# alexcoca/DistributedKernelShap

Measured on AMD Instinct MI355X. Metric: explanations/sec (2560 inst, 100-sample background), higher is better.
Workload: dtype fp32; 1 GPU; model=adult-logreg (12 groups, D=50, n_out=2, logit link), global_batch=2560, background=100, nsamples=default(2M+2048), parallelism=dp1, device=cuda

## Files before the change

distributedkernelshap_amd/config.py:

```python
from __future__ import annotations

import dataclasses
from dataclasses import dataclass, field
from typing import Any, Dict, List, Optional, Union

__all__ = [
    "EngineConfig",
    "DistributedConfig",
    "ServeConfig",
    "BenchConfig",
    "KernelConfig",
    "Config",
]


@dataclass
class EngineConfig:

    link: str = "logit"
    seed: int = 0
    nsamples: Optional[int] = None
    l1_reg: Union[str, int, float, None] = "auto"
    device: str = "auto"
    chunk_rows: int = 1 << 20


@dataclass
class DistributedConfig:

    n_workers: Optional[int] = None
    batch_size: int = 1
    actor_cpu_fraction: float = 1.0
    backend: str = "auto"
    mp_context: Optional[str] = None

    def to_opts(self) -> Dict[str, Any]:
        d = {
            "n_workers": self.n_workers,
            "batch_size": self.batch_size,
            "actor_cpu_fraction": self.actor_cpu_fraction,
        }
        if self.mp_context:
            d["mp_context"] = self.mp_context
        return d


@dataclass
class ServeConfig:
    host: str = "127.0.0.1"
    port: int = 8800
    replicas: int = 1
    max_batch_size: int = 64
    max_wait_ms: float = 2.0


@dataclass
class KernelConfig:

    wls_mode: str = "auto"
    fused_predict: bool = True
    predict_dtype: str = "fp32"
    packed_mma: str = "auto"
    synth_chunk_rows: int = 1 << 21
    l1_device: bool = True
    module_autocast: str = "off"
    module_channels_last: bool = True


@dataclass
class BenchConfig:
    instances: int = 2560
    background: int = 100
    nruns: int = 5
    steps: int = 5
    warmup: int = 2
    batch_sizes: List[int] = field(default_factory=lambda: [1, 5, 10])
    results_dir: str = "results"
    assets_dir: str = "assets"


@dataclass
class Config:
    engine: EngineConfig = field(default_factory=EngineConfig)
    distributed: DistributedConfig = field(default_factory=DistributedConfig)
    serve: ServeConfig = field(default_factory=ServeConfig)
    kernels: KernelConfig = field(default_factory=KernelConfig)
    bench: BenchConfig = field(default_factory=BenchConfig)

    @classmethod
    def from_dict(cls, d: Dict[str, Any]) -> "Config":
        cfg = cls()
        for section, values in d.items():
            if not hasattr(cfg, section):
                raise KeyError(f"unknown config section '{section}'")
            sub = getattr(cfg, section)
            names = {f.name for f in dataclasses.fields(sub)}
            for k, v in values.items():
                if k not in names:
                    raise KeyError(f"unknown key '{section}.{k}'")
                setattr(sub, k, v)
        return cfg

    @classmethod
    def from_toml(cls, path: str) -> "Config":
        import tomli

        with open(path, "rb") as f:
            return cls.from_dict(tomli.load(f))

    def to_dict(self) -> Dict[str, Any]:
        return dataclasses.asdict(self)
```

distributedkernelshap_amd/ops/gpu_engine.py:

```python
from __future__ import annotations

import logging
from typing import List, Optional

import numpy as np

from . import load_extension
from ..core.sampler import CoalitionPlan

logger = logging.getLogger(__name__)

import os as _os
import time as _time

_TIMING = _os.environ.get("KSHAP_TIMING", "") == "1"


class _StageTimer:

    def __init__(self, torch_mod, enabled, sink=None):
        self.t = torch_mod
        self.enabled = enabled or sink is not None
        self.sink = sink
        self.last = _time.perf_counter() if self.enabled else 0.0
# ... 590 lines not shown
                else t.tensor(varying, dtype=t.int64, device=self.device))
        xv = self._x_part(X_dev)[:, vidx]
        bgv = self.bg_part[:, vidx]
        return xv.permute(0, 2, 1)[:, :, :, None] - bgv.permute(2, 1, 0)[None]

    def _ey_fused_linear(self, masks, X_dev, varying, vidx_t=None):
        t = self.torch
        b, s, m = masks.shape
        mpad = max(4, (m + 3) // 4 * 4)
        npad = (self.N + 15) // 16 * 16
        if vidx_t is None:
            vidx_t = t.tensor(varying, dtype=t.int64, device=self.device)
        act, oimg = self._act_oimg()
        diff = self._buf(f"diff{m}", (b, oimg, mpad, npad), zeroed=True)
        self.ext.build_diff_f32(
            self._x_part_img(X_dev, act), self._bg_part_img(act), vidx_t, diff
        )
        base = t.zeros(oimg, npad, device=self.device)
        base[:, : self.N] = self._base_img(act)
        wbg = t.zeros(npad, device=self.device)
        wbg[: self.N] = self.bg_w
        ey = self._buf("ey", (b, s, self.n_out))
        self.ext.fused_predict_linear(masks, diff, base, wbg, ey, act)
        return ey

    def _act_oimg(self):
        act = self.linear["act"]
        if act == 2 and self.n_out == 2:
            return 3, 1
        return act, self.n_out

    def _x_part_img(self, X_dev, act):
        xp = self._x_part(X_dev)
        if act == 3:
            return (xp[:, :, 1:2] - xp[:, :, 0:1]).contiguous()
        return xp

    def _bg_part_img(self, act):
        if act == 3:
            if not hasattr(self, "_bg_part_d"):
                self._bg_part_d = (
                    self.bg_part[:, :, 1:2] - self.bg_part[:, :, 0:1]
                ).contiguous()
            return self._bg_part_d
        return self.bg_part

    def _base_img(self, act):
        if act == 3:
            return (self.baseN[:, 1] - self.baseN[:, 0])[None, :]
        return self.baseN.T

    def _ey_fused_bf16(self, masks, X_dev, varying, vidx_t=None, packed=None):
        t = self.torch
        b, s, m = masks.shape
        npad = (self.N + 15) // 16 * 16
        split = 2 if self.engine.kernels.predict_dtype == "bf16x2" else 1
        if packed is not None:
            self.ext.pack_masks(masks, packed)
        if vidx_t is None:
            vidx_t = t.tensor(varying, dtype=t.int64, device=self.device)
        act, oimg = self._act_oimg()
        diffB = self._buf(
            f"diffB{m}", (b, split, oimg, npad, 40), t.bfloat16, zeroed=True
        )
        self.ext.build_diff_bf16(
            self._x_part_img(X_dev, act), self._bg_part_img(act), vidx_t, diffB
        )
        base = t.zeros(oimg, npad, device=self.device)
        base[:, : self.N] = self._base_img(act)
        wbg = t.zeros(npad, device=self.device)
        wbg[: self.N] = self.bg_w
        ey = self._buf("ey", (b, s, self.n_out))
        self.ext.fused_predict_bf16(masks, diffB, base, wbg, ey, act)
        return ey

    def _ey_fused_tiled(self, masks, X_dev, varying, vidx_t=None):
        t = self.torch
        b, s, m = masks.shape
        mpad = max(16, (m + 15) // 16 * 16)
        npad = (self.N + 15) // 16 * 16
        if vidx_t is None:
            vidx_t = t.tensor(varying, dtype=t.int64, device=self.device)
        act, oimg = self._act_oimg()
        diff = self._buf(f"difft{m}", (b, oimg, mpad, npad), zeroed=True)
        self.ext.build_diff_f32(
            self._x_part_img(X_dev, act), self._bg_part_img(act), vidx_t, diff
        )
        base = t.zeros(oimg, npad, device=self.device)
        base[:, : self.N] = self._base_img(act)
        wbg = t.zeros(npad, device=self.device)
        wbg[: self.N] = self.bg_w
        n_ntiles = (npad + 127) // 128
        partial = self._buf("ftpart", (b, n_ntiles, s, self.n_out))
        ey = self._buf("ey", (b, s, self.n_out))
        self.ext.fused_predict_tiled(masks, diff, base, wbg, partial, ey, act)
        return ey

    def _ey_linear_f64(self, masks, X_dev, varying, s_chunk=2048):
        t = self.torch
        b, s, m = masks.shape
        W = self.linear["W"].double()
        bias = self.linear["b"].double()
        bg = self.bg.double()
        X64 = X_dev.double()
        contrib_x = X64[:, :, None] * W.T[None, :, :]
        x_part = t.zeros(b, self.n_groups, self.n_out, dtype=t.float64,
                         device=self.device)
        x_part.index_add_(1, self.col_group, contrib_x)
        contrib_b = bg[:, :, None] * W.T[None, :, :]
        bg_part = t.zeros(self.N, self.n_groups, self.n_out, dtype=t.float64,
                          device=self.device)
        bg_part.index_add_(1, self.col_group, contrib_b)
        vidx = t.tensor(varying, dtype=t.int64, device=self.device)
        diff = (x_part[:, vidx].permute(0, 2, 1)[:, :, :, None]
                - bg_part[:, vidx].permute(2, 1, 0)[None])
        diff = diff.permute(0, 2, 3, 1).reshape(b, m, self.N * self.n_out)
        base = bg @ W.T + bias
        wbg64 = self.bg_w.double()
        ey = t.empty(b, s, self.n_out, dtype=t.float64, device=self.device)
        for lo in range(0, s, s_chunk):
            hi = min(lo + s_chunk, s)
            logits = t.bmm(masks[:, lo:hi].double(), diff)
            logits = logits.view(b, hi - lo, self.N, self.n_out) + base[None, None]
            a = self.linear["act"]
            if a == 1:
                p = t.sigmoid(logits)
            elif a == 2:
                p = t.softmax(logits, dim=-1)
            else:
                p = logits
            ey[:, lo:hi] = t.einsum("bsno,n->bso", p, wbg64)
        return ey

    def _ey_fused_tiled_bf16(self, masks, X_dev, varying, vidx_t=None):
        t = self.torch
        b, s, m = masks.shape
        mpad = max(32, (m + 31) // 32 * 32)
        npad = (self.N + 15) // 16 * 16
        if vidx_t is None:
            vidx_t = t.tensor(varying, dtype=t.int64, device=self.device)
        act, oimg = self._act_oimg()
        split = 2 if self.engine.kernels.predict_dtype == "bf16x2" else 1
        diffb = self._buf(
            f"difftb{m}", (b, split, oimg, npad, mpad), t.bfloat16,
            zeroed=True,
        )
        self.ext.build_diff_bf16_tiled(
            self._x_part_img(X_dev, act), self._bg_part_img(act), vidx_t,
            diffb,
        )
        base = t.zeros(oimg, npad, device=self.device)
        base[:, : self.N] = self._base_img(act)
        wbg = t.zeros(npad, device=self.device)
        wbg[: self.N] = self.bg_w
        n_ntiles = (npad + 127) // 128
        partial = self._buf("ftpart", (b, n_ntiles, s, self.n_out))
        ey = self._buf("ey", (b, s, self.n_out))
        self.ext.fused_predict_tiled_bf16(
            masks, diffb, base, wbg, partial, ey, act
        )
        return ey

    def _ey_linear_torch(self, masks, X_dev, varying, s_chunk=4096):
        t = self.torch
        b, s, m = masks.shape
        diff = self._diff_tensor(X_dev, varying)
        diff = diff.permute(0, 2, 3, 1).reshape(b, m, self.N * self.n_out)
        ey = t.empty(b, s, self.n_out, device=self.device)
        for lo in range(0, s, s_chunk):
            hi = min(lo + s_chunk, s)
            logits = t.bmm(masks[:, lo:hi].float(), diff)
            logits = logits.view(b, hi - lo, self.N, self.n_out) + self.baseN[None, None]
            a = self.linear["act"]
            if a == 1:
                p = t.sigmoid(logits)
            elif a == 2:
                p = t.softmax(logits, dim=-1)
            else:
                p = logits
            ey[:, lo:hi] = t.einsum("bsno,n->bso", p, self.bg_w)
        return ey

    def _ey_torch_module(self, masks, X_dev, varying, chunk_rows=None):
        t = self.torch
        b, s, m = masks.shape
        if chunk_rows is None:
            chunk_rows = max(self.N, self.engine.kernels.synth_chunk_rows or 1 << 19)
        chunk_rows = min(chunk_rows, max(self.N, (1 << 29) // max(1, self.D)))
        chunk_rows = min(chunk_rows, b * s * self.N)
        ey = t.empty(b, s, self.n_out, device=self.device)
        vmap = np.full(self.n_groups, m, dtype=np.int64)
        for i, g in enumerate(varying):
            vmap[g] = i
        mfull = self._buf("mfull", (b, s, m + 1), t.uint8)
        mfull.zero_()
        mfull[:, :, :m] = masks
        colg = t.tensor(
            vmap[self.engine._col_group].astype(np.int32), device=self.device
        )
        sdt = (t.bfloat16 if self.engine.kernels.module_autocast == "bf16"
               else t.float32)
        rows_per_inst = s * self.N
        if rows_per_inst <= chunk_rows:
            g_inst = max(1, min(b, chunk_rows // rows_per_inst))
            buf = self._buf("synth", (g_inst * rows_per_inst, self.D), sdt)
            for lo in range(0, b, g_inst):
                hi = min(lo + g_inst, b)
                rows = (hi - lo) * rows_per_inst
                out = buf[:rows]
                self.ext.synth_chunk(mfull, X_dev, self.bg, colg, out, lo, hi, 0, s)
                y = self._predict_rows(out)
                ey[lo:hi] = t.einsum(
                    "csno,n->cso",
                    y.view(hi - lo, s, self.N, self.n_out),
                    self.bg_w,
                )
        else:
            s_chunk = max(1, chunk_rows // self.N)
            buf = self._buf("synth", (s_chunk * self.N, self.D), sdt)
            for bi in range(b):
                for lo in range(0, s, s_chunk):
                    hi = min(lo + s_chunk, s)
                    rows = (hi - lo) * self.N
                    out = buf[:rows]
                    self.ext.synth_chunk(
                        mfull, X_dev, self.bg, colg, out, bi, bi + 1, lo, hi
                    )
                    y = self._predict_rows(out)
                    y = y.view(hi - lo, self.N, self.n_out)
                    ey[bi, lo:hi] = t.einsum("cno,n->co", y, self.bg_w)
        return ey


    def _packed_ok(self, m, plan, l1_reg) -> bool:
        kc = self.engine.kernels
        return (
            self.linear is not None
            and kc.predict_dtype == "fp32"
            and kc.fused_predict
            and kc.wls_mode in ("auto", "mfma")
            and 2 <= m <= 64
            and (self.N + 15) // 16 * 16 <= 128
            and self.n_out in (1, 2, 4)
            and (m - 1) + self.n_out <= 16
            and not self._l1_active(plan, l1_reg)
        )

    def _packed_consts(self):
        c = getattr(self, "_packed_c", None)
        if c is None:
            t = self.torch
            act, oimg = self._act_oimg()
            npad = (self.N + 15) // 16 * 16
            base = t.zeros(oimg, npad, device=self.device)
            base[:, : self.N] = self._base_img(act)
            wbg = t.zeros(npad, device=self.device)
            wbg[: self.N] = self.bg_w
            lfnull64 = self._link(self.fnull.double()).contiguous()
            c = {
                "act": act, "oimg": oimg, "npad": npad, "base": base,
                "wbg": wbg, "lfnull64": lfnull64,
                "lfnull": lfnull64.float().contiguous(),
                "bgp": self._bg_part_img(act).contiguous(),
                "link": 0 if self.link_name == "identity" else 1,
            }
            self._packed_c = c
        return c

    def _packed_plan(self, plan):
        t = self.torch
        key = ("packed", plan.m, plan.nsamples)
        ent = self._enum_cache.get(key)
        if ent is None:
            ne = plan.enum_masks.shape[0]
            enum_packed = t.empty(1, ne, dtype=t.int64, device=self.device)
            if ne > 0:
                enum = t.tensor(plan.enum_masks, dtype=t.uint8,
                                device=self.device)
                self.ext.pack_masks(enum[None].contiguous(), enum_packed)
            kw = t.empty(plan.nsamples, dtype=t.float32, device=self.device)
            kw[:ne] = t.tensor(plan.enum_weights, dtype=t.float32,
                               device=self.device)
            if plan.n_random > 0:
                kw[ne:] = plan.weight_left / plan.n_random
            cdf = t.tensor(
                np.cumsum(plan.random_size_probs).astype(np.float32),
                device=self.device,
            )
            szs = t.tensor(plan.random_sizes.astype(np.int32),
                           device=self.device)
            ent = (enum_packed[0].contiguous(), kw, cdf, szs)
            self._enum_cache[key] = ent
        return ent

    def _packed_mma(self):
        mode = self.engine.kernels.packed_mma
        try:
            return {"auto": -1, "f32": 0, "split": 1}[mode]
        except KeyError:
            raise ValueError(
                f"packed_mma must be 'auto', 'f32' or 'split', got {mode!r}"
            ) from None

    def _packed_pipeline(self, X_dev, plan, vidx_t, ids_dev, phi_full,
                         timer=None):
        t = self.torch
        b = X_dev.shape[0]
        m, s = plan.m, plan.nsamples
        c = self._packed_consts()
        enum_packed, kw, cdf, szs = self._packed_plan(plan)
        mpad = max(4, (m + 3) // 4 * 4)
        packed = self._buf("packed", (b, s), t.int64)
        self.ext.fill_masks_packed(
            packed, enum_packed, plan.n_random, cdf, szs,
            int(np.floor((m - 1) / 2.0)), int(self.engine.seed), ids_dev, m,
        )
        if timer is not None:
            timer.mark("masks")
        diff = self._buf(f"diffp{m}", (b, c["oimg"], mpad, c["npad"]))
        total = self._buf("totalp", (b, self.n_out))
        self.ext.linear_prepare(
            X_dev, self.linear["W"], self.linear["b"], self.col_group, vidx_t,
            c["bgp"], c["lfnull64"], diff, total, c["act"], c["link"],
        )
        ey = self._buf("ey", (b, s, self.n_out))
        self.ext.fused_predict_linear_packed(
            packed, diff, c["base"], c["wbg"], ey, c["act"], c["link"],
            c["lfnull"], self._packed_mma(),
        )
        if timer is not None:
            timer.mark("predict")
        self.ext.wls_solve_packed(packed, kw, ey, total, vidx_t, phi_full)
        if timer is not None:
            timer.mark("wls")


    def _fused_body(self, X_dev, plan, varying, vidx_t, ids_dev, phi_full):
        t = self.torch
        b = X_dev.shape[0]
        m = len(varying)
        if self._packed_ok(m, plan, False):
            self._packed_pipeline(X_dev, plan, vidx_t, ids_dev, phi_full)
            return
        fx = self._predict_rows_f64(X_dev)
        lfx = self._link(fx)
        lfnull64 = self._link(self.fnull.double())
        total = (lfx - lfnull64[None, :]).float().contiguous()
        lfnull = lfnull64.float()
        masks, kw = self._device_masks(plan, np.arange(b), ids_dev=ids_dev)
        kc = self.engine.kernels
        packed = self._buf("packed", (b, plan.nsamples), t.int64)
        self.ext.pack_masks(masks, packed)
        if (kc.predict_dtype in ("bf16", "bf16x2") and m <= 32
                and self.n_out in (1, 2, 4)):
            ey = self._ey_fused_bf16(masks, X_dev, varying, vidx_t, packed=None)
        else:
            ey = self._ey_fused_linear(masks, X_dev, varying, vidx_t)
        if self.link_name == "identity":
            ey_adj = ey.sub_(lfnull[None, None, :])
        else:
            ey.clamp_(_EPS, 1.0 - _EPS)
            ey.log_().sub_(t.log1p(-t.exp(ey)))
            ey_adj = ey.sub_(lfnull[None, None, :])
        phi = self._buf("phi", (b, m, self.n_out))
        self.ext.wls_solve(masks, kw, ey_adj, total, phi, packed)
        phi_full.zero_()
        phi_full[:, vidx_t] = phi

    def _graph_explain(self, X_dev, plan, varying, instance_offset,
                       as_tensor=False):
        t = self.torch
        b = X_dev.shape[0]
        key = (b, plan.nsamples, varying.tobytes())
        entry = self._graphs.get(key)
        if entry is None:
            hits = self._graph_hits.get(key, 0) + 1
            self._graph_hits[key] = hits
            if hits < self._graph_min_hits or len(self._graphs) >= 8:
                return None
            try:
                vidx_t = t.tensor(varying, dtype=t.int64, device=self.device)
                x_static = self._buf("Xg", (b, self.D))
                ids_static = self._buf("idsg", (b,), t.int32)
                phi_full = t.zeros(
                    b, self.n_groups, self.n_out, device=self.device
                )
                x_static.copy_(X_dev)
                ids_static.copy_(
                    t.arange(instance_offset, instance_offset + b,
                             dtype=t.int32, device=self.device)
                )
                side = t.cuda.Stream()
                side.wait_stream(t.cuda.current_stream())
                with t.cuda.stream(side):
                    self._fused_body(
                        x_static, plan, varying, vidx_t, ids_static, phi_full
                    )
                t.cuda.current_stream().wait_stream(side)
                graph = t.cuda.CUDAGraph()
                with t.cuda.graph(graph):
                    self._fused_body(
                        x_static, plan, varying, vidx_t, ids_static, phi_full
                    )
                entry = (graph, x_static, ids_static, phi_full, vidx_t)
                self._graphs[key] = entry
            except Exception as e:
                logger.warning(
                    "hipGraph capture failed (%r); continuing eagerly", e
                )
                self._graphs_enabled = False
                return None
        graph, x_static, ids_static, phi_full, _ = entry
        if x_static.data_ptr() != X_dev.data_ptr():
            x_static.copy_(X_dev)
        ids_static.copy_(
            t.arange(instance_offset, instance_offset + b, dtype=t.int32,
                     device=self.device)
        )
        graph.replay()
        if as_tensor:
            return phi_full.clone()
        out = phi_full.double().cpu().numpy()
        return [np.ascontiguousarray(out[:, :, o]) for o in range(self.n_out)]

    _CHUNK_BYTES = 2 << 30

    def _instances_per_chunk(self, nsamples: Optional[int],
                             l1_reg="auto") -> int:
        from ..core.sampler import default_nsamples

        s = nsamples or default_nsamples(max(2, self.n_groups))
        g = self.n_groups
        if g >= 2 and self._packed_ok(g, self.engine._plan(g, nsamples),
                                      l1_reg):
            npad = (self.N + 15) // 16 * 16
            per_inst = (s * (8 + 4 * self.n_out)
                        + 4 * self.n_out * (g + 3) * npad + (1 << 14))
            return max(1, self._CHUNK_BYTES // per_inst)
        npad = (self.N + 15) // 16 * 16
        n_ntiles = (npad + 127) // 128
        per_inst = s * (g + 8 + 4 + 4 * self.n_out) + (1 << 14)
        if g > 64 or npad > 128:
            per_inst += s * 4 * self.n_out * n_ntiles
            mpad = max(4, (g + 3) // 4 * 4)
            per_inst += 4 * mpad * npad * max(1, self.n_out)
            per_inst += 8 * g * (g + self.n_out) * 2
        if self.mlp_fused:
            h1 = self.mlp["pack"]["hpad"][0]
            per_inst += 8 * g * (self.D + 2 * h1) + 4 * h1 * (g + 31)
        if self.trees_kernel == "bits":
            per_inst += self.trees["pack"]["n_trees"] * (8 + 64 * 9)
        return max(1, self._CHUNK_BYTES // per_inst)

    def shap_values(
        self,
        X: np.ndarray,
        nsamples: Optional[int] = None,
        l1_reg="auto",
        instance_offset: int = 0,
        as_tensor: bool = False,
    ) -> List[np.ndarray]:
        t = self.torch
        b_total = X.shape[0]
        chunk = self._instances_per_chunk(nsamples, l1_reg)
        if b_total > chunk:
            if as_tensor:
                out = t.empty(
                    b_total, self.n_groups, self.n_out, device=self.device,
                    dtype=(t.float64
                           if self.engine.kernels.predict_dtype == "fp64"
                           else t.float32),
                )
                for lo in range(0, b_total, chunk):
                    hi = min(lo + chunk, b_total)
                    out[lo:hi] = self.shap_values(
                        X[lo:hi], nsamples=nsamples, l1_reg=l1_reg,
                        instance_offset=instance_offset + lo, as_tensor=True,
                    )
                return out
            parts = [
                self.shap_values(
                    X[lo : lo + chunk], nsamples=nsamples, l1_reg=l1_reg,
                    instance_offset=instance_offset + lo,
                )
                for lo in range(0, b_total, chunk)
            ]
            return [
                np.concatenate([p[o] for p in parts], axis=0)
                for o in range(self.n_out)
            ]
        timer = _StageTimer(t, _TIMING, sink=self.trace)
        if t.is_tensor(X):
            b = X.shape[0]
            if X.is_cuda:
                X_dev = X.float()
            else:
                X_dev = self._spec_x_static(b, X.shape[1])
                if X_dev is None:
                    X_dev = self._buf("X", (b, X.shape[1]))
                X_dev.copy_(X, non_blocking=True)
        else:
            X = np.ascontiguousarray(X, dtype=np.float64)
            b = X.shape[0]
            X_dev = t.tensor(X, dtype=t.float32, device=self.device)
        timer.mark("h2d")

        fp64 = self.engine.kernels.predict_dtype == "fp64"
        if (
            self._graphs_enabled
            and not fp64
            and self._spec is not None
            and self.linear is not None
            and self.n_groups <= 62
        ):
            sk0, skey, sm = self._spec
            sb, sns, soff = skey[0], skey[1], skey[3]
            entry = self._graphs.get((skey[0], skey[1], skey[2]))
            spec_plan = self.engine._plan(sm, nsamples) if entry is not None else None
            if (entry is not None and sb == b and spec_plan.nsamples == sns
                    and not self._l1_active(spec_plan, l1_reg)
                    and soff == int(instance_offset)):
                graph, x_static, ids_static, gphi, _ = entry
                if x_static.data_ptr() != X_dev.data_ptr():
                    x_static.copy_(X_dev)
                graph.replay()
                _, probe = self._varying_probe(x_static)
                staged = None if as_tensor else self._phi_stage_enqueue(gphi)
                pc = probe.cpu()
                timer.mark("spec")
                if bool(pc[0]) and int(pc[1]) == sk0:
                    if as_tensor:
                        return gphi.clone()
                    timer.mark("d2h")
                    return [
                        np.ascontiguousarray(staged[:, :, o], dtype=np.float64)
                        for o in range(self.n_out)
                    ]
                self._spec = None

        X64_dev = None
        f64c = next((c for c in (self.mlp, self.trees, self.km)
                     if c is not None), None)
        if fp64 and f64c is not None:
            X64_dev = (X.to(self.device).double() if t.is_tensor(X)
                       else t.tensor(X, dtype=t.float64, device=self.device))
        fx = self._predict_rows_f64(
            X_dev if X64_dev is None else X64_dev)
        lfx = self._link(fx)
        lfnull64 = self._link(
            self.fnull.double() if X64_dev is None else f64c["fnull64"])
        total_all = (lfx - lfnull64[None, :])
        if not fp64:
            total_all = total_all.float()
        lfnull = lfnull64.float()

        phi_full = t.zeros(b, self.n_groups, self.n_out, device=self.device,
                           dtype=t.float64 if fp64 else t.float32)

        if self.n_groups <= 62:
            keys, probe = self._varying_probe(X_dev)
            probe = probe.cpu()
            timer.mark("varying")
            if bool(probe[0]):
                key0 = int(probe[1])
                uniq = np.array(
                    [[(key0 >> g) & 1 for g in range(self.n_groups)]],
                    dtype=bool,
                )
                inverse = np.zeros(b, dtype=np.int64)
            else:
                ks = keys.cpu().numpy()
                kuniq, inverse = np.unique(ks, return_inverse=True)
                uniq = ((kuniq[:, None] >> np.arange(self.n_groups)) & 1
                        ).astype(bool)
        else:
            vmat = self._varying_matrix_dev(X_dev).cpu().numpy()
            timer.mark("varying")
            uniq, inverse = np.unique(vmat, axis=0, return_inverse=True)
        timer.mark("bucket")

        kc = self.engine.kernels
        if self._graphs_enabled and not fp64 and uniq.shape[0] == 1 \
                and self.linear is not None \
                and kc.fused_predict and kc.wls_mode in ("auto", "mfma"):
            varying0 = np.nonzero(uniq[0])[0]
            m0 = len(varying0)
            if m0 >= 2:
                plan0 = self.engine._plan(m0, nsamples)
                mpad0 = max(4, (m0 + 3) // 4 * 4)
                npad0 = (self.N + 15) // 16 * 16
                if (
                    mpad0 <= 64
                    and npad0 <= 128
                    and self.n_out in (1, 2, 4)
                    and not self._l1_active(plan0, l1_reg)
                ):
                    out = self._graph_explain(
                        X_dev, plan0, varying0, instance_offset,
                        as_tensor=as_tensor,
                    )
                    if out is not None:
                        key0 = 0
                        for g in varying0:
                            key0 |= 1 << int(g)
                        self._spec = (
                            key0,
                            (b, plan0.nsamples, varying0.tobytes(),
                             int(instance_offset)),
                            m0,
                        )
                        timer.mark("graph")
                        return out

        for u in range(uniq.shape[0]):
            varying = np.nonzero(uniq[u])[0]
            m = len(varying)
            ids = np.nonzero(inverse == u)[0]
            ids_t = t.tensor(ids, dtype=t.int64, device=self.device)
            if m == 0:
                continue
            if m == 1:
                phi_full[ids_t, int(varying[0])] = total_all[ids_t]
                continue
            plan = self.engine._plan(m, nsamples)
            gids = ids + instance_offset
            if not fp64 and self._packed_ok(m, plan, l1_reg):
                nb = len(ids)
# ... 364 lines not shown
```

distributedkernelshap_amd/ops/hip/bindings.cpp:

```cpp
#include <torch/extension.h>
#include <ATen/hip/HIPContext.h>
#include <c10/hip/HIPStream.h>

#include <cstdint>

extern "C" void launch_fill_random_masks(
    uint8_t* masks, int B, int S, int M, int ne, int n_random,
    const float* cdf, const int* sizes, int n_sizes, int num_paired,
    uint32_t seed, const int32_t* inst_ids, hipStream_t stream);

extern "C" int launch_fused_predict_linear(
    const uint8_t* masksU, const float* diff, const float* base, const float* wbg,
    float* ey, int B, int S, int M, int Mpad, int Npad, int n_out, int act,
    hipStream_t stream);

extern "C" void launch_synth_chunk(
    const uint8_t* masks, const float* x, const float* bg, const int* col_group,
    void* out, int out_bf16, int S, int M, int N, int D, int b_lo, int b_hi,
    int s_lo, int s_hi, hipStream_t stream);

extern "C" void launch_pack_masks(
    const uint8_t* masks, uint64_t* packed, int B, int S, int M,
    hipStream_t stream);

extern "C" int launch_fused_predict_bf16(
    const uint8_t* masksU, const uint16_t* diffB,
    const float* base, const float* wbg, float* ey, int B, int S, int M,
    int Npad, int n_out, int act, int split, hipStream_t stream);

extern "C" void launch_build_diff_f32(
    const float* xp, const float* bgp, const int64_t* vidx, float* out,
    int B, int G, int O, int N, int m, int Mpad, int Npad, hipStream_t stream);

extern "C" void launch_build_diff_bf16(
    const float* xp, const float* bgp, const int64_t* vidx, uint16_t* out,
    int B, int G, int O, int N, int m, int Npad, int split, hipStream_t stream);

extern "C" int launch_wls_solve(
    const uint8_t* masks, const uint64_t* packed, const float* kw,
    const float* ey_adj, const float* total, float* phi, int B, int S, int M,
    int n_out, hipStream_t stream);

extern "C" void launch_pack_masks_words(
    const uint8_t* masks, uint64_t* packed, int B, int S, int M, int W,
    hipStream_t stream);

extern "C" int launch_wls_gram(
    const uint64_t* packed, const float* kw, const float* ey_adj,
    const float* total, double* A64, double* rhs64, int B, int S, int M,
    int W, int n_out, hipStream_t stream);

extern "C" int launch_fused_predict_tiled(
    const uint8_t* masksU, const float* diff, const float* base,
    const float* wbg, float* partial, float* ey, int B, int S, int M,
    int Mpad, int Npad, int n_out, int act, hipStream_t stream);

extern "C" void launch_build_diff_bf16_tiled(
    const float* xp, const float* bgp, const int64_t* vidx, uint16_t* out,
    int B, int G, int O, int N, int m, int Mpad, int Npad, int split,
    hipStream_t stream);

extern "C" int launch_fused_predict_tiled_bf16(
    const uint8_t* masksU, const uint16_t* diffB, const float* base,
    const float* wbg, float* partial, float* ey, int B, int S, int M,
    int Mpad, int Npad, int n_out, int act, int split, hipStream_t stream);

extern "C" int launch_fill_masks_packed(
    uint64_t* packed, const uint64_t* enum_packed, int B, int S, int M, int ne,
    int n_random, const float* cdf, const int* sizes, int n_sizes,
    int num_paired, uint32_t seed, const int32_t* inst_ids, hipStream_t stream);

extern "C" int launch_linear_prepare(
    const float* X, const float* W, const float* bias,
    const int64_t* col_group, const int64_t* vidx, const float* bgp,
    const double* lfnull64, float* diff, float* total, int B, int D, int G,
    int N, int m, int Mpad, int Npad, int n_out, int act, int link,
    hipStream_t stream);

extern "C" int launch_fused_predict_linear_packed(
    const uint64_t* packed, const float* diff, const float* base,
    const float* wbg, const float* lfnull, float* ey, int B, int S, int Mpad,
    int Npad, int n_out, int act, int link, hipStream_t stream, int mma);

extern "C" int launch_wls_solve_packed(
    const uint64_t* packed, const float* kw, const float* ey_adj,
    const float* total, const int64_t* vidx, float* phi_full, int B, int S,
    int M, int n_out, int G, hipStream_t stream);

extern "C" int launch_varying_probe(
    const float* X, const float* bg_min, const float* bg_max,
    const float* tol_min, const float* tol_max, const int64_t* col_group,
    int64_t* keys, int64_t* probe, int B, int D, int G, hipStream_t stream);

extern "C" int launch_fused_predict_mlp(
    const uint8_t* masks, const void* xp1, const void* bgp1n,
    const float* base1, const void* const* hw, const float* const* hb,
    const int* H, int nhid, const void* wout, const float* bout,
    const float* wbg, float* ey, int B, int S, int M, int Mpad, int N,
    int n_out, int act, int hidden_act, int is_bf16, int nsplit,
    hipStream_t stream);

extern "C" int launch_fused_predict_trees(
    const uint8_t* masks, const int* vmap, const int64_t* dx, const int64_t* dbg,
    const uint8_t* child, const int* meta, const float* leaves,
    const int* grp_off, const int* grp_id, const int64_t* grp_mask,
    const float* base, const float* wbg, float* ey, float scale,
    int B, int S, int Mv, int N, int T, int G, int E, int L, int C,
    int max_internal, int n_out, int act, int leaf_mode, hipStream_t stream);

extern "C" int launch_fused_predict_trees_walk(
    const uint8_t* masks, const int* vmap, const float* x, const float* bg,
    const int* nodes, const int* roots, const float* leaves, const float* base,
    const float* wbg, float* ey, float scale,
    int B, int S, int Mv, int N, int D, int G, int T, int R, int L,
    int max_depth, int n_out, int act, int leaf_mode,
    const unsigned* cat_left, int C, hipStream_t stream);

extern "C" int launch_fused_predict_kernelmachine(
    const uint8_t* masks, const float* xp, const float* bgpn,
    const float* base, const float* alpha, const float* icpt,
    const float* wbg, float* ey, int B, int S, int M, int Mpad, int N,
    int Vpad, int n_out, int act, int kernel, float gamma, float coef0,
    int degree, hipStream_t stream);

namespace {

#define CHECK_DEV(t) TORCH_CHECK((t).is_cuda() && (t).is_contiguous(), #t " must be a contiguous device tensor")

hipStream_t current_stream() {
    return c10::hip::getCurrentHIPStream().stream();
}

void fill_random_masks(
    torch::Tensor masks, int64_t ne, int64_t n_random,
    torch::Tensor cdf, torch::Tensor sizes, int64_t num_paired, int64_t seed,
    torch::Tensor inst_ids) {
    CHECK_DEV(masks); CHECK_DEV(cdf); CHECK_DEV(sizes); CHECK_DEV(inst_ids);
    TORCH_CHECK(masks.dtype() == torch::kUInt8, "masks must be uint8");
    TORCH_CHECK(masks.dim() == 3, "masks must be (B,S,M)");
    TORCH_CHECK(inst_ids.dtype() == torch::kInt32, "inst_ids must be int32");
    int B = masks.size(0), S = masks.size(1), M = masks.size(2);
    TORCH_CHECK(inst_ids.size(0) == B, "inst_ids length");
    TORCH_CHECK(M <= 256, "fill_random_masks supports M <= 256");
    launch_fill_random_masks(
        masks.data_ptr<uint8_t>(), B, S, M, (int)ne, (int)n_random,
        cdf.data_ptr<float>(), sizes.data_ptr<int>(), (int)cdf.size(0),
        (int)num_paired, (uint32_t)seed, inst_ids.data_ptr<int32_t>(),
        current_stream());
}

void fused_predict_linear(
    torch::Tensor masks, torch::Tensor diff, torch::Tensor base,
    torch::Tensor wbg, torch::Tensor ey, int64_t act) {
    CHECK_DEV(masks); CHECK_DEV(diff); CHECK_DEV(base); CHECK_DEV(wbg); CHECK_DEV(ey);
    TORCH_CHECK(masks.dtype() == torch::kUInt8, "masks must be u8 (B,S,M)");
    int B = masks.size(0), S = masks.size(1), M = masks.size(2);
    int Mpad = diff.size(2), Npad = diff.size(3);
    int n_out = ey.size(2);
    int oimg = (act == 3) ? 1 : n_out;
    TORCH_CHECK(diff.size(1) == oimg, "diff image count vs act");
    TORCH_CHECK(M <= Mpad, "M vs Mpad");
    TORCH_CHECK(ey.size(0) == B && ey.size(1) == S, "ey shape");
    TORCH_CHECK(base.size(0) == oimg && base.size(1) == Npad, "base shape");
    TORCH_CHECK(wbg.size(0) == Npad, "wbg shape");
    int rc = launch_fused_predict_linear(
        masks.data_ptr<uint8_t>(), diff.data_ptr<float>(), base.data_ptr<float>(),
        wbg.data_ptr<float>(), ey.data_ptr<float>(), B, S, M, Mpad, Npad,
        n_out, (int)act, current_stream());
    TORCH_CHECK(rc == 0, "fused_predict_linear: unsupported shape (Mpad<=64, Npad%16==0, Npad<=128, n_out in {1,2,4})");
}

void synth_chunk(
    torch::Tensor masks, torch::Tensor x, torch::Tensor bg,
    torch::Tensor col_group, torch::Tensor out, int64_t b_lo, int64_t b_hi,
    int64_t s_lo, int64_t s_hi) {
    CHECK_DEV(masks); CHECK_DEV(x); CHECK_DEV(bg); CHECK_DEV(col_group); CHECK_DEV(out);
    int S = masks.size(1), M = masks.size(2);
    int N = bg.size(0), D = bg.size(1);
    TORCH_CHECK(out.size(0) == (b_hi - b_lo) * (s_hi - s_lo) * N && out.size(1) == D,
                "out shape");
    const bool bf16 = out.dtype() == torch::kBFloat16;
    TORCH_CHECK(bf16 || out.dtype() == torch::kFloat32,
                "out must be float32 or bfloat16");
    launch_synth_chunk(
        masks.data_ptr<uint8_t>(), x.data_ptr<float>(), bg.data_ptr<float>(),
        col_group.data_ptr<int>(),
        bf16 ? (void*)out.data_ptr<at::BFloat16>()
             : (void*)out.data_ptr<float>(),
        bf16 ? 1 : 0, S, M, N, D,
        (int)b_lo, (int)b_hi, (int)s_lo, (int)s_hi, current_stream());
}

void wls_solve(
    torch::Tensor masks, torch::Tensor kw, torch::Tensor ey_adj,
    torch::Tensor total, torch::Tensor phi,
    c10::optional<torch::Tensor> packed) {
    CHECK_DEV(masks); CHECK_DEV(kw); CHECK_DEV(ey_adj); CHECK_DEV(total); CHECK_DEV(phi);
    int B = masks.size(0), S = masks.size(1), M = masks.size(2);
    int n_out = ey_adj.size(2);
    TORCH_CHECK(phi.size(0) == B && phi.size(1) == M && phi.size(2) == n_out, "phi shape");
    const uint64_t* pk = nullptr;
    if (packed.has_value()) {
        CHECK_DEV(packed.value());
        TORCH_CHECK(packed->size(0) == B && packed->size(1) == S, "packed shape");
        pk = reinterpret_cast<const uint64_t*>(packed->data_ptr<int64_t>());
    }
    int rc = launch_wls_solve(
        masks.data_ptr<uint8_t>(), pk, kw.data_ptr<float>(), ey_adj.data_ptr<float>(),
        total.data_ptr<float>(), phi.data_ptr<float>(), B, S, M, n_out,
        current_stream());
    TORCH_CHECK(rc == 0, "wls_solve: unsupported shape (2<=M<=64, n_out<=8)");
}

void pack_masks(torch::Tensor masks, torch::Tensor packed) {
    CHECK_DEV(masks); CHECK_DEV(packed);
    TORCH_CHECK(masks.dtype() == torch::kUInt8, "masks must be u8");
    int B = masks.size(0), S = masks.size(1), M = masks.size(2);
    TORCH_CHECK(M <= 64, "pack_masks supports M <= 64");
    TORCH_CHECK(packed.size(0) == B && packed.size(1) == S, "packed shape");
    launch_pack_masks(
        masks.data_ptr<uint8_t>(),
        reinterpret_cast<uint64_t*>(packed.data_ptr<int64_t>()),
        B, S, M, current_stream());
}

#define CHECK_F32(t) TORCH_CHECK((t).dtype() == torch::kFloat32, #t " must be float32")
#define CHECK_I64(t) TORCH_CHECK((t).dtype() == torch::kInt64, #t " must be int64")

void fill_masks_packed(
    torch::Tensor packed, torch::Tensor enum_packed, int64_t n_random,
    torch::Tensor cdf, torch::Tensor sizes, int64_t num_paired, int64_t seed,
    torch::Tensor inst_ids, int64_t M) {
    CHECK_DEV(packed); CHECK_DEV(enum_packed); CHECK_DEV(cdf); CHECK_DEV(sizes);
    CHECK_DEV(inst_ids);
    CHECK_I64(packed); CHECK_I64(enum_packed); CHECK_F32(cdf);
    TORCH_CHECK(sizes.dtype() == torch::kInt32, "sizes must be int32");
    TORCH_CHECK(inst_ids.dtype() == torch::kInt32, "inst_ids must be int32");
    TORCH_CHECK(packed.dim() == 2 && enum_packed.dim() == 1,
                "packed must be (B,S), enum_packed (ne,)");
    int B = packed.size(0), S = packed.size(1), ne = enum_packed.size(0);
    TORCH_CHECK(inst_ids.dim() == 1 && inst_ids.size(0) == B, "inst_ids length");
    TORCH_CHECK(n_random >= 0 && ne + n_random == S, "ne + n_random must equal S");
    TORCH_CHECK(cdf.dim() == 1 && sizes.dim() == 1
                && cdf.size(0) == sizes.size(0), "cdf vs sizes");
    TORCH_CHECK(n_random == 0 || cdf.size(0) >= 1, "empty size table");
    int rc = launch_fill_masks_packed(
        reinterpret_cast<uint64_t*>(packed.data_ptr<int64_t>()),
        reinterpret_cast<const uint64_t*>(enum_packed.data_ptr<int64_t>()),
        B, S, (int)M, ne, (int)n_random, cdf.data_ptr<float>(),
        sizes.data_ptr<int>(), (int)cdf.size(0), (int)num_paired,
        (uint32_t)seed, inst_ids.data_ptr<int32_t>(), current_stream());
    TORCH_CHECK(rc == 0, "fill_masks_packed: unsupported shape (1<=M<=64)");
}

void linear_prepare(
    torch::Tensor X, torch::Tensor W, torch::Tensor bias,
    torch::Tensor col_group, torch::Tensor vidx, torch::Tensor bgp,
    torch::Tensor lfnull64, torch::Tensor diff, torch::Tensor total,
    int64_t act, int64_t link) {
    CHECK_DEV(X); CHECK_DEV(W); CHECK_DEV(bias); CHECK_DEV(col_group);
    CHECK_DEV(vidx); CHECK_DEV(bgp); CHECK_DEV(lfnull64); CHECK_DEV(diff);
    CHECK_DEV(total);
    CHECK_F32(X); CHECK_F32(W); CHECK_F32(bias); CHECK_F32(bgp); CHECK_F32(diff);
    CHECK_F32(total); CHECK_I64(col_group); CHECK_I64(vidx);
    TORCH_CHECK(lfnull64.dtype() == torch::kFloat64, "lfnull64 must be float64");
    TORCH_CHECK(X.dim() == 2 && W.dim() == 2 && bgp.dim() == 3 && diff.dim() == 4
                && total.dim() == 2 && vidx.dim() == 1, "operand ranks");
    int B = X.size(0), D = X.size(1), n_out = W.size(0);
    int N = bgp.size(0), G = bgp.size(1), OI = bgp.size(2), m = vidx.size(0);
    int Mpad = diff.size(2), Npad = diff.size(3);
    TORCH_CHECK(W.size(1) == D && bias.numel() == n_out
                && col_group.numel() == D && lfnull64.numel() == n_out,
                "W (n_out,D), b (n_out), col_group (D), lfnull64 (n_out)");
    TORCH_CHECK(OI == (act == 3 ? 1 : n_out), "background image count vs act");
    TORCH_CHECK(diff.size(0) == B && diff.size(1) == OI, "diff (B,OI,Mpad,Npad)");
    TORCH_CHECK(total.size(0) == B && total.size(1) == n_out, "total (B,n_out)");
    TORCH_CHECK(link == 0 || link == 1, "link must be 0 or 1");
    int rc = launch_linear_prepare(
        X.data_ptr<float>(), W.data_ptr<float>(), bias.data_ptr<float>(),
        col_group.data_ptr<int64_t>(), vidx.data_ptr<int64_t>(),
        bgp.data_ptr<float>(), lfnull64.data_ptr<double>(),
        diff.data_ptr<float>(), total.data_ptr<float>(), B, D, G, N, m, Mpad,
        Npad, n_out, (int)act, (int)link, current_stream());
    TORCH_CHECK(rc == 0, "linear_prepare: unsupported shape (m<=Mpad, m<=64, "
                         "N<=Npad, n_out<=8, act 3 needs n_out==2)");
}

void fused_predict_linear_packed(
    torch::Tensor packed, torch::Tensor diff, torch::Tensor base,
    torch::Tensor wbg, torch::Tensor ey, int64_t act, int64_t link,
    c10::optional<torch::Tensor> lfnull, int64_t mma) {
    CHECK_DEV(packed); CHECK_DEV(diff); CHECK_DEV(base); CHECK_DEV(wbg); CHECK_DEV(ey);
    CHECK_I64(packed); CHECK_F32(diff); CHECK_F32(base); CHECK_F32(wbg); CHECK_F32(ey);
    TORCH_CHECK(packed.dim() == 2 && diff.dim() == 4 && ey.dim() == 3
                && base.dim() == 2, "operand ranks");
    int B = packed.size(0), S = packed.size(1);
    int Mpad = diff.size(2), Npad = diff.size(3);
    int n_out = ey.size(2);
    int oimg = (act == 3) ? 1 : n_out;
    TORCH_CHECK(diff.size(0) == B && diff.size(1) == oimg, "diff (B,oimg,Mpad,Npad) vs act");
    TORCH_CHECK(ey.size(0) == B && ey.size(1) == S, "ey shape");
    TORCH_CHECK(base.size(0) == oimg && base.size(1) == Npad, "base shape");
    TORCH_CHECK(wbg.numel() == Npad, "wbg shape");
    const float* lf = nullptr;
    if (lfnull.has_value()) {
        CHECK_DEV(lfnull.value()); CHECK_F32(lfnull.value());
        TORCH_CHECK(lfnull->numel() == n_out, "lfnull must be (n_out,)");
        lf = lfnull->data_ptr<float>();
    }
    TORCH_CHECK(link == 0 || (link == 1 && lf != nullptr),
                "link must be 0, or 1 with lfnull given");
    TORCH_CHECK(mma >= -1 && mma <= 1,
                "mma must be -1 (auto), 0 (fp32 MFMA) or 1 (split bf16 MFMA)");
    int rc = launch_fused_predict_linear_packed(
        reinterpret_cast<const uint64_t*>(packed.data_ptr<int64_t>()),
        diff.data_ptr<float>(), base.data_ptr<float>(), wbg.data_ptr<float>(),
        lf, ey.data_ptr<float>(), B, S, Mpad, Npad, n_out, (int)act, (int)link,
        current_stream(), (int)mma);
    TORCH_CHECK(rc == 0, "fused_predict_linear_packed: unsupported shape "
                         "(Mpad%4==0, Mpad<=64, Npad%16==0, Npad<=128, n_out in "
                         "{1,2,4}, operand images within 64 KiB of LDS)");
}

void wls_solve_packed(
    torch::Tensor packed, torch::Tensor kw, torch::Tensor ey_adj,
    torch::Tensor total, torch::Tensor vidx, torch::Tensor phi_full) {
    CHECK_DEV(packed); CHECK_DEV(kw); CHECK_DEV(ey_adj); CHECK_DEV(total);
    CHECK_DEV(vidx); CHECK_DEV(phi_full);
    CHECK_I64(packed); CHECK_F32(kw); CHECK_F32(ey_adj); CHECK_F32(total);
    CHECK_I64(vidx); CHECK_F32(phi_full);
    TORCH_CHECK(packed.dim() == 2 && ey_adj.dim() == 3 && phi_full.dim() == 3
                && vidx.dim() == 1 && total.dim() == 2, "operand ranks");
    int B = packed.size(0), S = packed.size(1), M = vidx.size(0);
    int n_out = ey_adj.size(2), G = phi_full.size(1);
    TORCH_CHECK(kw.numel() == S, "kw must be (S,)");
    TORCH_CHECK(ey_adj.size(0) == B && ey_adj.size(1) == S, "ey_adj shape");
    TORCH_CHECK(total.size(0) == B && total.size(1) == n_out, "total shape");
    TORCH_CHECK(phi_full.size(0) == B && phi_full.size(2) == n_out, "phi_full shape");
    int rc = launch_wls_solve_packed(
        reinterpret_cast<const uint64_t*>(packed.data_ptr<int64_t>()),
        kw.data_ptr<float>(), ey_adj.data_ptr<float>(), total.data_ptr<float>(),
        vidx.data_ptr<int64_t>(), phi_full.data_ptr<float>(), B, S, M, n_out,
        G, current_stream());
    TORCH_CHECK(rc == 0, "wls_solve_packed: unsupported shape (2<=M<=G, "
                         "(M-1)+n_out<=16)");
}

void varying_probe(
    torch::Tensor X, torch::Tensor bg_min, torch::Tensor bg_max,
    torch::Tensor tol_min, torch::Tensor tol_max, torch::Tensor col_group,
    int64_t n_groups, torch::Tensor keys, torch::Tensor probe) {
    CHECK_DEV(X); CHECK_DEV(bg_min); CHECK_DEV(bg_max); CHECK_DEV(tol_min);
    CHECK_DEV(tol_max); CHECK_DEV(col_group); CHECK_DEV(keys); CHECK_DEV(probe);
    CHECK_F32(X); CHECK_F32(bg_min); CHECK_F32(bg_max); CHECK_F32(tol_min);
    CHECK_F32(tol_max); CHECK_I64(col_group); CHECK_I64(keys); CHECK_I64(probe);
    TORCH_CHECK(X.dim() == 2, "X must be (B,D)");
    const int64_t B = X.size(0), D = X.size(1);
    TORCH_CHECK(B >= 1 && D >= 1 && B <= 0x7fffffffLL && D <= 0x7fffffffLL,
                "X must be (B,D) with B, D >= 1");
    TORCH_CHECK(bg_min.numel() == D && bg_max.numel() == D
                && tol_min.numel() == D && tol_max.numel() == D
                && col_group.numel() == D,
                "bg_min, bg_max, tol_min, tol_max, col_group must be (D,)");
    TORCH_CHECK(keys.numel() == B, "keys must be (B,)");
    TORCH_CHECK(probe.numel() == 2, "probe must be (2,)");
    int rc = launch_varying_probe(
        X.data_ptr<float>(), bg_min.data_ptr<float>(), bg_max.data_ptr<float>(),
        tol_min.data_ptr<float>(), tol_max.data_ptr<float>(),
        col_group.data_ptr<int64_t>(), keys.data_ptr<int64_t>(),
        probe.data_ptr<int64_t>(), (int)B, (int)D, (int)n_groups,
        current_stream());
    TORCH_CHECK(rc == 0, "varying_probe: unsupported shape (1 <= n_groups <= 62)");
}

void fused_predict_bf16(
    torch::Tensor masks, torch::Tensor diffB, torch::Tensor base,
    torch::Tensor wbg, torch::Tensor ey, int64_t act) {
    CHECK_DEV(masks); CHECK_DEV(diffB); CHECK_DEV(base); CHECK_DEV(wbg); CHECK_DEV(ey);
    TORCH_CHECK(masks.dtype() == torch::kUInt8 && diffB.dtype() == torch::kBFloat16);
    int B = masks.size(0), S = masks.size(1), M = masks.size(2);
    int split = diffB.size(1), Npad = diffB.size(3);
    int n_out = ey.size(2);
    TORCH_CHECK(diffB.size(2) == ((act == 3) ? 1 : n_out), "diffB image count vs act");
    TORCH_CHECK(diffB.size(0) == B && diffB.size(4) == 40, "diffB (B,split,o,Npad,40)");
    TORCH_CHECK(ey.size(0) == B && ey.size(1) == S, "ey shape");
    int rc = launch_fused_predict_bf16(
        masks.data_ptr<uint8_t>(),
        reinterpret_cast<const uint16_t*>(diffB.data_ptr<at::BFloat16>()),
        base.data_ptr<float>(), wbg.data_ptr<float>(), ey.data_ptr<float>(),
        B, S, M, Npad, n_out, (int)act, split, current_stream());
    TORCH_CHECK(rc == 0, "fused_predict_bf16: unsupported shape (M<=32, Npad<=128, n_out in {1,2,4}, split in {1,2})");
}

void build_diff_f32(torch::Tensor xp, torch::Tensor bgp, torch::Tensor vidx,
                    torch::Tensor out) {
    CHECK_DEV(xp); CHECK_DEV(bgp); CHECK_DEV(vidx); CHECK_DEV(out);
    int B = xp.size(0), G = xp.size(1), O = xp.size(2);
    int N = bgp.size(0), m = vidx.size(0);
    int Mpad = out.size(2), Npad = out.size(3);
    TORCH_CHECK(out.size(0) == B && out.size(1) == O && m <= Mpad && N <= Npad);
    launch_build_diff_f32(
        xp.data_ptr<float>(), bgp.data_ptr<float>(), vidx.data_ptr<int64_t>(),
        out.data_ptr<float>(), B, G, O, N, m, Mpad, Npad, current_stream());
}

void build_diff_bf16(torch::Tensor xp, torch::Tensor bgp, torch::Tensor vidx,
                     torch::Tensor out) {
    CHECK_DEV(xp); CHECK_DEV(bgp); CHECK_DEV(vidx); CHECK_DEV(out);
    TORCH_CHECK(out.dtype() == torch::kBFloat16 && out.size(4) == 40);
    int B = xp.size(0), G = xp.size(1), O = xp.size(2);
    int N = bgp.size(0), m = vidx.size(0);
    int split = out.size(1), Npad = out.size(3);
    TORCH_CHECK(out.size(0) == B && out.size(2) == O && N <= Npad && m <= 32);
    launch_build_diff_bf16(
        xp.data_ptr<float>(), bgp.data_ptr<float>(), vidx.data_ptr<int64_t>(),
        reinterpret_cast<uint16_t*>(out.data_ptr<at::BFloat16>()), B, G, O, N,
        m, Npad, split, current_stream());
}

void pack_masks_words(torch::Tensor masks, torch::Tensor packed) {
    CHECK_DEV(masks); CHECK_DEV(packed);
    TORCH_CHECK(masks.dtype() == torch::kUInt8, "masks must be u8");
    TORCH_CHECK(packed.dim() == 3, "packed must be (B,S,W)");
    int B = masks.size(0), S = masks.size(1), M = masks.size(2);
    int W = packed.size(2);
    TORCH_CHECK(packed.size(0) == B && packed.size(1) == S, "packed shape");
    TORCH_CHECK(W * 64 >= M, "packed word count vs M");
    launch_pack_masks_words(
        masks.data_ptr<uint8_t>(),
        reinterpret_cast<uint64_t*>(packed.data_ptr<int64_t>()),
        B, S, M, W, current_stream());
}

void wls_gram(
    torch::Tensor packed, torch::Tensor kw, torch::Tensor ey_adj,
    torch::Tensor total, torch::Tensor A64, torch::Tensor rhs64) {
    CHECK_DEV(packed); CHECK_DEV(kw); CHECK_DEV(ey_adj); CHECK_DEV(total);
    CHECK_DEV(A64); CHECK_DEV(rhs64);
    TORCH_CHECK(packed.dim() == 3, "packed must be (B,S,W)");
    TORCH_CHECK(A64.dtype() == torch::kFloat64 && rhs64.dtype() == torch::kFloat64);
    int B = packed.size(0), S = packed.size(1), W = packed.size(2);
    int mm = A64.size(1), n_out = ey_adj.size(2);
    TORCH_CHECK(A64.size(0) == B && A64.size(2) == mm, "A64 shape");
    TORCH_CHECK(rhs64.size(0) == B && rhs64.size(1) == mm
                && rhs64.size(2) == n_out, "rhs64 shape");
    TORCH_CHECK(W * 64 >= mm + 1, "packed word count vs M");
    int rc = launch_wls_gram(
        reinterpret_cast<const uint64_t*>(packed.data_ptr<int64_t>()),
        kw.data_ptr<float>(), ey_adj.data_ptr<float>(),
        total.data_ptr<float>(), A64.data_ptr<double>(),
        rhs64.data_ptr<double>(), B, S, mm + 1, W, n_out, current_stream());
    TORCH_CHECK(rc == 0, "wls_gram: unsupported shape (M<=513, n_out<=8)");
}

void fused_predict_tiled(
    torch::Tensor masks, torch::Tensor diff, torch::Tensor base,
    torch::Tensor wbg, torch::Tensor partial, torch::Tensor ey, int64_t act) {
    CHECK_DEV(masks); CHECK_DEV(diff); CHECK_DEV(base); CHECK_DEV(wbg);
    CHECK_DEV(partial); CHECK_DEV(ey);
    TORCH_CHECK(masks.dtype() == torch::kUInt8, "masks must be u8 (B,S,M)");
    int B = masks.size(0), S = masks.size(1), M = masks.size(2);
    int Mpad = diff.size(2), Npad = diff.size(3);
    int n_out = ey.size(2);
    int oimg = (act == 3) ? 1 : n_out;
    int nacc = n_out;
    int n_ntiles = (Npad + 127) / 128;
    TORCH_CHECK(diff.size(1) == oimg, "diff image count vs act");
    TORCH_CHECK(M <= Mpad, "M vs Mpad");
    TORCH_CHECK(ey.size(0) == B && ey.size(1) == S, "ey shape");
    TORCH_CHECK(base.size(0) == oimg && base.size(1) == Npad, "base shape");
    TORCH_CHECK(wbg.size(0) == Npad, "wbg shape");
    TORCH_CHECK(partial.size(0) == B && partial.size(1) == n_ntiles
                && partial.size(2) == S && partial.size(3) == nacc,
                "partial shape (B, n_ntiles, S, nacc)");
    int rc = launch_fused_predict_tiled(
        masks.data_ptr<uint8_t>(), diff.data_ptr<float>(),
        base.data_ptr<float>(), wbg.data_ptr<float>(),
        partial.data_ptr<float>(), ey.data_ptr<float>(), B, S, M, Mpad,
        Npad, n_out, (int)act, current_stream());
    TORCH_CHECK(rc == 0, "fused_predict_tiled: unsupported shape "
                         "(Mpad%4==0, Npad%16==0, n_out in {1,2,4})");
}

void build_diff_bf16_tiled(torch::Tensor xp, torch::Tensor bgp,
                           torch::Tensor vidx, torch::Tensor out) {
    CHECK_DEV(xp); CHECK_DEV(bgp); CHECK_DEV(vidx); CHECK_DEV(out);
    TORCH_CHECK(out.dtype() == torch::kBFloat16 && out.dim() == 5,
                "out must be bf16 (B,split,O,Npad,Mpad)");
    int B = xp.size(0), G = xp.size(1), O = xp.size(2);
    int N = bgp.size(0), mcount = vidx.size(0);
    int split = out.size(1), Npad = out.size(3), Mpad = out.size(4);
    TORCH_CHECK(out.size(0) == B && out.size(2) == O && N <= Npad
                && mcount <= Mpad);
    launch_build_diff_bf16_tiled(
        xp.data_ptr<float>(), bgp.data_ptr<float>(), vidx.data_ptr<int64_t>(),
        reinterpret_cast<uint16_t*>(out.data_ptr<at::BFloat16>()), B, G, O, N,
        mcount, Mpad, Npad, split, current_stream());
}

void fused_predict_tiled_bf16(
    torch::Tensor masks, torch::Tensor diffB, torch::Tensor base,
    torch::Tensor wbg, torch::Tensor partial, torch::Tensor ey, int64_t act) {
    CHECK_DEV(masks); CHECK_DEV(diffB); CHECK_DEV(base); CHECK_DEV(wbg);
    CHECK_DEV(partial); CHECK_DEV(ey);
    TORCH_CHECK(masks.dtype() == torch::kUInt8
                && diffB.dtype() == torch::kBFloat16);
    int B = masks.size(0), S = masks.size(1), M = masks.size(2);
    int split = diffB.size(1), Npad = diffB.size(3), Mpad = diffB.size(4);
    int n_out = ey.size(2);
    int oimg = (act == 3) ? 1 : n_out;
    int n_ntiles = (Npad + 127) / 128;
    TORCH_CHECK(diffB.size(2) == oimg, "diffB image count vs act");
    TORCH_CHECK(ey.size(0) == B && ey.size(1) == S, "ey shape");
    TORCH_CHECK(base.size(0) == oimg && base.size(1) == Npad, "base shape");
    TORCH_CHECK(wbg.size(0) == Npad, "wbg shape");
    TORCH_CHECK(partial.size(0) == B && partial.size(1) == n_ntiles
                && partial.size(2) == S && partial.size(3) == n_out,
                "partial shape");
    TORCH_CHECK((size_t)split * oimg * 128 * 40 * 2 <= 64 * 1024,
                "bf16 tiled LDS footprint (split*oimg too large)");
    int rc = launch_fused_predict_tiled_bf16(
        masks.data_ptr<uint8_t>(),
        reinterpret_cast<const uint16_t*>(diffB.data_ptr<at::BFloat16>()),
        base.data_ptr<float>(), wbg.data_ptr<float>(),
        partial.data_ptr<float>(), ey.data_ptr<float>(), B, S, M, Mpad, Npad,
        n_out, (int)act, split, current_stream());
    TORCH_CHECK(rc == 0, "fused_predict_tiled_bf16: unsupported shape "
                         "(Mpad%32==0, Npad%16==0, n_out in {1,2,4})");
}

void fused_predict_mlp(
    torch::Tensor masks, torch::Tensor xp1, torch::Tensor bgp1n,
    torch::Tensor base1, std::vector<torch::Tensor> hidden_w,
    std::vector<torch::Tensor> hidden_b, torch::Tensor wout,
    torch::Tensor bout, torch::Tensor wbg, torch::Tensor ey, int64_t act,
    int64_t hidden_act) {
    static const char* envelope =
        "fused_predict_mlp: outside the supported envelope (1-3 relu hidden "
        "layers of padded width <= 256, n_out <= 8, M <= Mpad <= 64, widths "
        "padded to 16 (fp32) / 32 (bf16))";
    CHECK_DEV(masks); CHECK_DEV(xp1); CHECK_DEV(bgp1n); CHECK_DEV(base1);
    CHECK_DEV(wout); CHECK_DEV(bout); CHECK_DEV(wbg); CHECK_DEV(ey);
    TORCH_CHECK(masks.dtype() == torch::kUInt8 && masks.dim() == 3,
                "masks must be u8 (B,S,M)");
    const bool bf16 = xp1.dtype() == torch::kBFloat16;
    TORCH_CHECK(bf16 || xp1.dtype() == torch::kFloat32,
                "operand images must be float32 or bfloat16");
    const auto wdt = xp1.dtype();
    TORCH_CHECK(hidden_w.size() == hidden_b.size(), "hidden_w vs hidden_b");
    TORCH_CHECK(hidden_w.size() + 1 <= 3, envelope);
    const int nhid = (int)hidden_w.size() + 1;
    TORCH_CHECK(xp1.dim() == 3 && bgp1n.dim() == 3 && base1.dim() == 2
                && wout.dim() == 3 && ey.dim() == 3, "operand ranks");
    int B = masks.size(0), S = masks.size(1), M = masks.size(2);
    int H[3] = {(int)xp1.size(1), 0, 0};
    int Mpad = xp1.size(2), N = bgp1n.size(0), n_out = ey.size(2);
    TORCH_CHECK(xp1.size(0) == B, "xp1 must be (B,H1,Mpad)");
    TORCH_CHECK(bgp1n.dtype() == wdt && bgp1n.size(1) == H[0]
                && bgp1n.size(2) == Mpad, "bgp1n must be (N,H1,Mpad)");
    TORCH_CHECK(base1.dtype() == torch::kFloat32 && base1.size(0) == N
                && base1.size(1) == H[0], "base1 must be f32 (N,H1)");
    const void* hw[2] = {nullptr, nullptr};
    const float* hb[2] = {nullptr, nullptr};
    for (int l = 1; l < nhid; ++l) {
        const torch::Tensor& w = hidden_w[l - 1];
        const torch::Tensor& bb = hidden_b[l - 1];
        CHECK_DEV(w); CHECK_DEV(bb);
        TORCH_CHECK(w.dtype() == wdt && w.dim() == 2 && w.size(1) == H[l - 1],
                    "hidden weight must be (H_out, H_in) in the operand dtype");
        H[l] = w.size(0);
        TORCH_CHECK(bb.dtype() == torch::kFloat32 && bb.dim() == 1
                    && bb.size(0) == H[l], "hidden bias must be f32 (H_out)");
        hw[l - 1] = w.data_ptr();
        hb[l - 1] = bb.data_ptr<float>();
    }
    const int nsplit = wout.size(0);
    TORCH_CHECK(wout.dtype() == wdt && wout.size(1) == 16
                && wout.size(2) == H[nhid - 1], "wout must be (nsplit,16,H_last)");
    TORCH_CHECK(bout.dtype() == torch::kFloat32 && bout.numel() == 16,
                "bout must be f32 (16)");
    TORCH_CHECK(wbg.dtype() == torch::kFloat32 && wbg.numel() == N, "wbg must be f32 (N)");
    TORCH_CHECK(ey.dtype() == torch::kFloat32 && ey.size(0) == B
                && ey.size(1) == S, "ey must be f32 (B,S,n_out)");
    int rc = launch_fused_predict_mlp(
        masks.data_ptr<uint8_t>(), xp1.data_ptr(), bgp1n.data_ptr(),
        base1.data_ptr<float>(), hw, hb, H, nhid, wout.data_ptr(),
        bout.data_ptr<float>(), wbg.data_ptr<float>(), ey.data_ptr<float>(),
        B, S, M, Mpad, N, n_out, (int)act, (int)hidden_act, bf16 ? 1 : 0,
        nsplit, current_stream());
    TORCH_CHECK(rc != -2, "fused_predict_mlp: LDS size attribute rejected");
    TORCH_CHECK(rc == 0, envelope);
}

void fused_predict_trees(
    torch::Tensor masks, torch::Tensor vmap, torch::Tensor dx,
    torch::Tensor dbg, torch::Tensor child, torch::Tensor meta,
    torch::Tensor leaves, torch::Tensor grp_off, torch::Tensor grp_id,
    torch::Tensor grp_mask, torch::Tensor base, double scale,
    torch::Tensor wbg, torch::Tensor ey, int64_t act, int64_t leaf_mode,
    int64_t max_internal) {
    static const char* envelope =
        "fused_predict_trees: outside the supported envelope (1-1024 trees of "
        "at most 64 internal nodes each, n_out <= 8, 128 B per tree plus 2 B "
        "per internal node within 160 KiB of LDS)";
    CHECK_DEV(masks); CHECK_DEV(vmap); CHECK_DEV(dx); CHECK_DEV(dbg);
    CHECK_DEV(child); CHECK_DEV(meta); CHECK_DEV(leaves); CHECK_DEV(grp_off);
    CHECK_DEV(grp_id); CHECK_DEV(grp_mask); CHECK_DEV(base); CHECK_DEV(wbg);
    CHECK_DEV(ey);
    TORCH_CHECK(masks.dtype() == torch::kUInt8 && masks.dim() == 3,
                "masks must be u8 (B,S,Mv)");
    TORCH_CHECK(ey.dtype() == torch::kFloat32 && ey.dim() == 3,
                "ey must be f32 (B,S,n_out)");
    const int B = masks.size(0), S = masks.size(1), Mv = masks.size(2);
    const int n_out = ey.size(2);
    TORCH_CHECK(ey.size(0) == B && ey.size(1) == S, "ey must be f32 (B,S,n_out)");
    TORCH_CHECK(vmap.dtype() == torch::kInt32 && vmap.dim() == 1,
                "the group table must be int32 (G)");
    TORCH_CHECK(dx.dtype() == torch::kInt64 && dx.dim() == 2 && dx.size(0) == B,
                "dx must be int64 (B,T)");
    const int T = dx.size(1);
    TORCH_CHECK(dbg.dtype() == torch::kInt64 && dbg.dim() == 2
                && dbg.size(1) == T, "dbg must be int64 (N,T)");
    const int N = dbg.size(0);
    TORCH_CHECK(child.dtype() == torch::kUInt8 && child.dim() == 2
                && child.size(1) == 2, "child must be u8 (C,2)");
    TORCH_CHECK(meta.dtype() == torch::kInt32 && meta.dim() == 2
                && meta.size(0) == T && meta.size(1) == 4,
                "meta must be int32 (T,4)");
    TORCH_CHECK(leaf_mode == 0 || leaf_mode == 1, "leaf_mode must be 0 or 1");
    TORCH_CHECK(leaves.dtype() == torch::kFloat32
                && (leaf_mode == 0 ? leaves.dim() == 1
                                   : (leaves.dim() == 2 && leaves.size(1) == n_out)),
                "leaves must be f32 (L) for scalar or (L,n_out) for vector leaves");
    TORCH_CHECK(grp_off.dtype() == torch::kInt32 && grp_off.dim() == 1
                && grp_off.size(0) == T + 1, "grp_off must be int32 (T+1)");
    TORCH_CHECK(grp_id.dtype() == torch::kInt32 && grp_id.dim() == 1,
                "grp_id must be int32 (E)");
    TORCH_CHECK(grp_mask.dtype() == torch::kInt64 && grp_mask.dim() == 1
                && grp_mask.size(0) == grp_id.size(0), "grp_mask must be int64 (E)");
    TORCH_CHECK(base.dtype() == torch::kFloat32 && base.numel() == n_out,
                "base must be f32 (n_out)");
    TORCH_CHECK(wbg.dtype() == torch::kFloat32 && wbg.numel() == N,
                "wbg must be f32 (N)");
    TORCH_CHECK(max_internal <= 64 && max_internal >= 1, envelope);
    int rc = launch_fused_predict_trees(
        masks.data_ptr<uint8_t>(), vmap.data_ptr<int>(), dx.data_ptr<int64_t>(),
        dbg.data_ptr<int64_t>(), child.data_ptr<uint8_t>(), meta.data_ptr<int>(),
        leaves.data_ptr<float>(), grp_off.data_ptr<int>(), grp_id.data_ptr<int>(),
        grp_mask.data_ptr<int64_t>(), base.data_ptr<float>(),
        wbg.data_ptr<float>(), ey.data_ptr<float>(), (float)scale, B, S, Mv, N,
        T, (int)vmap.size(0), (int)grp_id.size(0), (int)leaves.size(0),
        (int)child.size(0), (int)max_internal, n_out, (int)act, (int)leaf_mode,
        current_stream());
    TORCH_CHECK(rc != -2, "fused_predict_trees: LDS size attribute rejected");
    TORCH_CHECK(rc == 0, envelope);
}

void fused_predict_trees_walk(
    torch::Tensor masks, torch::Tensor vmap, torch::Tensor x, torch::Tensor bg,
    torch::Tensor nodes, torch::Tensor roots, torch::Tensor leaves,
    torch::Tensor base, double scale, torch::Tensor wbg, torch::Tensor ey,
    int64_t act, int64_t leaf_mode, int64_t max_depth,
    c10::optional<torch::Tensor> cat_left) {
    static const char* envelope =
        "fused_predict_trees_walk: outside the supported envelope (depth <= "
        "64, n_out <= 8, at most 1024 groups and 4096 features, node records "
        "indexed by int32)";
    CHECK_DEV(masks); CHECK_DEV(vmap); CHECK_DEV(x); CHECK_DEV(bg);
    CHECK_DEV(nodes); CHECK_DEV(roots); CHECK_DEV(leaves); CHECK_DEV(base);
    CHECK_DEV(wbg); CHECK_DEV(ey);
    TORCH_CHECK(masks.dtype() == torch::kUInt8 && masks.dim() == 3,
                "masks must be u8 (B,S,Mv)");
    TORCH_CHECK(ey.dtype() == torch::kFloat32 && ey.dim() == 3,
                "ey must be f32 (B,S,n_out)");
    const int B = masks.size(0), S = masks.size(1), Mv = masks.size(2);
    const int n_out = ey.size(2);
    TORCH_CHECK(ey.size(0) == B && ey.size(1) == S, "ey must be f32 (B,S,n_out)");
    TORCH_CHECK(vmap.dtype() == torch::kInt32 && vmap.dim() == 1,
                "the group table must be int32 (G)");
    TORCH_CHECK(x.dtype() == torch::kFloat32 && x.dim() == 2 && x.size(0) == B,
                "x must be f32 (B,D)");
    const int64_t D = x.size(1);
    TORCH_CHECK(bg.dtype() == torch::kFloat32 && bg.dim() == 2
                && bg.size(1) == D, "bg must be f32 (N,D)");
    const int N = bg.size(0);
    TORCH_CHECK(nodes.dtype() == torch::kInt32 && nodes.dim() == 2
                && nodes.size(1) == 4, "nodes must be int32 (R,4)");
    TORCH_CHECK(roots.dtype() == torch::kInt32 && roots.dim() == 1,
                "roots must be int32 (T)");
    TORCH_CHECK(leaf_mode == 0 || leaf_mode == 1, "leaf_mode must be 0 or 1");
    TORCH_CHECK(leaves.dtype() == torch::kFloat32
                && (leaf_mode == 0 ? leaves.dim() == 1
                                   : (leaves.dim() == 2 && leaves.size(1) == n_out)),
                "leaves must be f32 (L) for scalar or (L,n_out) for vector leaves");
    TORCH_CHECK(base.dtype() == torch::kFloat32 && base.numel() == n_out,
                "base must be f32 (n_out)");
    TORCH_CHECK(wbg.dtype() == torch::kFloat32 && wbg.numel() == N,
                "wbg must be f32 (N)");
    TORCH_CHECK(max_depth >= 0 && max_depth <= 64, envelope);
    const unsigned* cat_ptr = nullptr;
    int64_t C = 0;
    if (cat_left.has_value()) {
        const torch::Tensor& cl = *cat_left;
        CHECK_DEV(cl);
        TORCH_CHECK(cl.dtype() == torch::kInt32 && cl.dim() == 2
                    && cl.size(1) == 8 && cl.size(0) >= 1,
                    "cat_left must be int32 (C,8) with C >= 1");
        TORCH_CHECK(cl.size(0) <= 0x7fffffffLL / 8, envelope);
        cat_ptr = reinterpret_cast<const unsigned*>(cl.data_ptr<int>());
        C = cl.size(0);
    }
    TORCH_CHECK(nodes.size(0) <= 0x7fffffffLL && leaves.size(0) <= 0x7fffffffLL
                && roots.size(0) <= 0x7fffffffLL && D <= 0x7fffffffLL
                && vmap.size(0) <= 0x7fffffffLL, envelope);
    int rc = launch_fused_predict_trees_walk(
        masks.data_ptr<uint8_t>(), vmap.data_ptr<int>(), x.data_ptr<float>(),
        bg.data_ptr<float>(), nodes.data_ptr<int>(), roots.data_ptr<int>(),
        leaves.data_ptr<float>(), base.data_ptr<float>(), wbg.data_ptr<float>(),
        ey.data_ptr<float>(), (float)scale, B, S, Mv, N, (int)D,
        (int)vmap.size(0), (int)roots.size(0), (int)nodes.size(0),
        (int)leaves.size(0), (int)max_depth, n_out, (int)act, (int)leaf_mode,
        cat_ptr, (int)C, current_stream());
    TORCH_CHECK(rc != -2, "fused_predict_trees_walk: LDS size attribute rejected");
    TORCH_CHECK(rc == 0, envelope);
}

void fused_predict_kernelmachine(
    torch::Tensor masks, torch::Tensor xp, torch::Tensor bgpn,
    torch::Tensor base, torch::Tensor alpha, torch::Tensor intercept,
    torch::Tensor wbg, torch::Tensor ey, int64_t kernel, double gamma,
    double coef0, int64_t degree, int64_t act) {
    static const char* envelope =
        "fused_predict_kernelmachine: outside the supported envelope (rbf or "
        "poly of degree 1-8, at most 2048 support vectors after padding to "
        "16, n_out <= 8, M <= Mpad <= 64 with Mpad a multiple of 16)";
    CHECK_DEV(masks); CHECK_DEV(xp); CHECK_DEV(bgpn); CHECK_DEV(base);
    CHECK_DEV(alpha); CHECK_DEV(intercept); CHECK_DEV(wbg); CHECK_DEV(ey);
    TORCH_CHECK(masks.dtype() == torch::kUInt8 && masks.dim() == 3,
                "masks must be u8 (B,S,M)");
    TORCH_CHECK(xp.dtype() == torch::kFloat32 && xp.dim() == 3,
                "xp must be f32 (B,Vpad,Mpad)");
    const int B = masks.size(0), S = masks.size(1), M = masks.size(2);
    const int Vpad = xp.size(1), Mpad = xp.size(2);
    TORCH_CHECK(xp.size(0) == B, "xp must be f32 (B,Vpad,Mpad)");
    TORCH_CHECK(bgpn.dtype() == torch::kFloat32 && bgpn.dim() == 3
                && bgpn.size(1) == Vpad && bgpn.size(2) == Mpad,
                "bgpn must be f32 (N,Vpad,Mpad)");
    const int N = bgpn.size(0);
    TORCH_CHECK(base.dtype() == torch::kFloat32 && base.dim() == 2
                && base.size(0) == N && base.size(1) == Vpad,
                "base must be f32 (N,Vpad)");
    TORCH_CHECK(alpha.dtype() == torch::kFloat32 && alpha.dim() == 2
                && alpha.size(0) == 16 && alpha.size(1) == Vpad,
                "alpha must be f32 (16,Vpad)");
    TORCH_CHECK(intercept.dtype() == torch::kFloat32 && intercept.numel() == 16,
                "intercept must be f32 (16)");
    TORCH_CHECK(wbg.dtype() == torch::kFloat32 && wbg.numel() == N,
                "wbg must be f32 (N)");
    TORCH_CHECK(ey.dtype() == torch::kFloat32 && ey.dim() == 3
                && ey.size(0) == B && ey.size(1) == S,
                "ey must be f32 (B,S,n_out)");
    const int n_out = ey.size(2);
    int rc = launch_fused_predict_kernelmachine(
        masks.data_ptr<uint8_t>(), xp.data_ptr<float>(), bgpn.data_ptr<float>(),
        base.data_ptr<float>(), alpha.data_ptr<float>(),
        intercept.data_ptr<float>(), wbg.data_ptr<float>(),
        ey.data_ptr<float>(), B, S, M, Mpad, N, Vpad, n_out, (int)act,
        (int)kernel, (float)gamma, (float)coef0, (int)degree, current_stream());
    TORCH_CHECK(rc == 0, envelope);
}

}

PYBIND11_MODULE(TORCH_EXTENSION_NAME, m) {
    m.def("fused_predict_kernelmachine", &fused_predict_kernelmachine,
          "fused kernel-machine predict (K4k): distance / dot product folded "
          "over varying groups, support vectors streamed in tiles of 16, "
          "kernel evaluation and the contraction with alpha on chip",
          pybind11::arg("masks"), pybind11::arg("xp"), pybind11::arg("bgpn"),
          pybind11::arg("base"), pybind11::arg("alpha"),
          pybind11::arg("intercept"), pybind11::arg("wbg"), pybind11::arg("ey"),
          pybind11::arg("kernel"), pybind11::arg("gamma"),
          pybind11::arg("coef0"), pybind11::arg("degree"), pybind11::arg("act"));
    m.def("fused_predict_trees", &fused_predict_trees,
          "fused tree-ensemble predict (K4t): per-tree node masks in LDS, "
          "bitwise select of packed x / background decisions, bit-register walk",
          pybind11::arg("masks"), pybind11::arg("vmap"), pybind11::arg("dx"),
          pybind11::arg("dbg"), pybind11::arg("child"), pybind11::arg("meta"),
          pybind11::arg("leaves"), pybind11::arg("grp_off"),
          pybind11::arg("grp_id"), pybind11::arg("grp_mask"),
          pybind11::arg("base"), pybind11::arg("scale"), pybind11::arg("wbg"),
          pybind11::arg("ey"), pybind11::arg("act"), pybind11::arg("leaf_mode"),
          pybind11::arg("max_internal"));
    m.def("fused_predict_trees_walk", &fused_predict_trees_walk,
          "fused deep-tree predict (K4w): 16-byte node records walked on the "
          "blended row, group bitset per sample, x row and background in LDS",
          pybind11::arg("masks"), pybind11::arg("vmap"), pybind11::arg("x"),
          pybind11::arg("bg"), pybind11::arg("nodes"), pybind11::arg("roots"),
          pybind11::arg("leaves"), pybind11::arg("base"),
          pybind11::arg("scale"), pybind11::arg("wbg"), pybind11::arg("ey"),
          pybind11::arg("act"), pybind11::arg("leaf_mode"),
          pybind11::arg("max_depth"),
          pybind11::arg("cat_left") = pybind11::none());
    m.def("fused_predict_mlp", &fused_predict_mlp,
          "fused MLP predict (K4m): first layer folded over varying groups, "
          "hidden activations in LDS, f32 or bf16 MFMA by operand dtype",
          pybind11::arg("masks"), pybind11::arg("xp1"), pybind11::arg("bgp1n"),
          pybind11::arg("base1"), pybind11::arg("hidden_w"),
          pybind11::arg("hidden_b"), pybind11::arg("wout"),
          pybind11::arg("bout"), pybind11::arg("wbg"), pybind11::arg("ey"),
          pybind11::arg("act"), pybind11::arg("hidden_act") = 0);
    m.def("fill_masks_packed", &fill_masks_packed,
          "Philox coalition sampling straight into packed u64 words (K2p): "
          "bit-identical to the enumerated-row copy, fill_random_masks and "
          "pack_masks in sequence, M <= 64",
          pybind11::arg("packed"), pybind11::arg("enum_packed"),
          pybind11::arg("n_random"), pybind11::arg("cdf"),
          pybind11::arg("sizes"), pybind11::arg("num_paired"),
          pybind11::arg("seed"), pybind11::arg("inst_ids"), pybind11::arg("M"));
    m.def("linear_prepare", &linear_prepare,
          "per-call operand prep for the packed linear pipeline (K0p): diff "
          "image in the build_diff_f32 layout plus the fp64-evaluated totals",
          pybind11::arg("X"), pybind11::arg("W"), pybind11::arg("b"),
          pybind11::arg("col_group"), pybind11::arg("vidx"),
          pybind11::arg("bgp"), pybind11::arg("lfnull64"),
          pybind11::arg("diff"), pybind11::arg("total"), pybind11::arg("act"),
          pybind11::arg("link"));
    m.def("fused_predict_linear_packed", &fused_predict_linear_packed,
          "MFMA fused predict from packed mask words with the link fused into "
          "the epilogue (K3p); mma: -1 auto, 0 fp32 MFMA, 1 split-operand bf16 "
          "MFMA (Mpad <= 12, act 1/3; other shapes take the fp32 MFMA path)",
          pybind11::arg("packed"), pybind11::arg("diff"), pybind11::arg("base"),
          pybind11::arg("wbg"), pybind11::arg("ey"), pybind11::arg("act"),
          pybind11::arg("link") = 0, pybind11::arg("lfnull") = pybind11::none(),
          pybind11::arg("mma") = -1);
    m.def("wls_solve_packed", &wls_solve_packed,
          "MFMA WLS solve with (S,) kernel weights, scattered into "
          "phi_full (B,G,n_out) through vidx (K7p)",
          pybind11::arg("packed"), pybind11::arg("kw"), pybind11::arg("ey_adj"),
          pybind11::arg("total"), pybind11::arg("vidx"),
          pybind11::arg("phi_full"));
    m.def("varying_probe", &varying_probe,
          "varying-pattern probe (K1p): per-instance group bit keys and "
          "[all(keys == keys[0]), keys[0]] in two launches, no host sync",
          pybind11::arg("X"), pybind11::arg("bg_min"), pybind11::arg("bg_max"),
          pybind11::arg("tol_min"), pybind11::arg("tol_max"),
          pybind11::arg("col_group"), pybind11::arg("n_groups"),
          pybind11::arg("keys"), pybind11::arg("probe"));
    m.def("fill_random_masks", &fill_random_masks,
          "Philox coalition sampling (K2)");
    m.def("fused_predict_linear", &fused_predict_linear,
          "MFMA fused mask@diff GEMM + activation + background reduce (K3-K6)");
    m.def("build_diff_f32", &build_diff_f32,
          "diff image in the f32 fused-kernel layout");
    m.def("build_diff_bf16", &build_diff_bf16,
          "hi(+lo) diff images in the bf16 fused-kernel layout");
    m.def("pack_masks", &pack_masks,
          "masks u8 -> packed u64 bits (for the MFMA WLS Gram build)");
    m.def("fused_predict_bf16", &fused_predict_bf16,
          "bf16 matrix-core fused predict (single or hi+lo split), A-operand "
          "converted in-register from the raw u8 masks");
    m.def("synth_chunk", &synth_chunk,
          "masked-background perturbation synthesis tile (K3')");
    m.def("wls_solve", &wls_solve,
          "batched constrained WLS Shapley solve (K7)",
          pybind11::arg("masks"), pybind11::arg("kw"), pybind11::arg("ey_adj"),
          pybind11::arg("total"), pybind11::arg("phi"),
          pybind11::arg("packed") = pybind11::none());
    m.def("pack_masks_words", &pack_masks_words,
          "masks u8 -> (B,S,W) packed u64 words (wide-M Gram build)");
    m.def("wls_gram", &wls_gram,
          "tiled MFMA Gram+rhs build (fp64 via chunked promotion) for the "
          "stress WLS shapes, M up to 513");
    m.def("fused_predict_tiled", &fused_predict_tiled,
          "tiled MFMA fused predict for Mpad>64 / Npad>128 (LDS-streamed "
          "diff chunks, per-column-tile partials + deterministic reduce)");
    m.def("build_diff_bf16_tiled", &build_diff_bf16_tiled,
          "hi(+lo) k-contiguous diff image for the bf16 tiled predict");
    m.def("fused_predict_tiled_bf16", &fused_predict_tiled_bf16,
          "bf16 matrix-core tiled fused predict (v_mfma_f32_16x16x32_bf16 "
          "per 32-deep k block; hi+lo split for fp32-grade)");
}
```

distributedkernelshap_amd/ops/hip/kshap_kernels.hip:

```cpp

#include <hip/hip_runtime.h>
#include <cstdint>
#include <type_traits>

#include "split_bf16.h"

#define WAVE 64


struct Philox {
    uint32_t ctr[4];
    uint32_t key[2];
    uint32_t buf[4];
    int idx;

    __device__ void init(uint32_t k0, uint32_t k1, uint32_t c0, uint32_t c1) {
        key[0] = k0; key[1] = k1;
        ctr[0] = c0; ctr[1] = c1; ctr[2] = 0; ctr[3] = 0;
        idx = 4;
    }
    __device__ static void round_(uint32_t c[4], const uint32_t k[2]) {
        const uint32_t M0 = 0xD2511F53u, M1 = 0xCD9E8D57u;
        uint64_t p0 = (uint64_t)M0 * c[0];
        uint64_t p1 = (uint64_t)M1 * c[2];
// ... 1790 lines not shown
}

extern "C" int launch_fused_predict_tiled_bf16(
    const uint8_t* masksU, const uint16_t* diffB_u, const float* base,
    const float* wbg, float* partial, float* ey, int B, int S, int M,
    int Mpad, int Npad, int n_out, int act, int split, hipStream_t stream)
{
    if (Npad % 16 != 0 || Mpad % FTB_KC != 0 || split < 1 || split > 2)
        return -1;
    const __bf16* diffB = reinterpret_cast<const __bf16*>(diffB_u);
    switch (n_out) {
        case 1: launch_ftb_act<1>(masksU, diffB, base, wbg, partial, ey, B, S, M, Mpad, Npad, act, split, stream); break;
        case 2: launch_ftb_act<2>(masksU, diffB, base, wbg, partial, ey, B, S, M, Mpad, Npad, act, split, stream); break;
        case 4: launch_ftb_act<4>(masksU, diffB, base, wbg, partial, ey, B, S, M, Mpad, Npad, act, split, stream); break;
        default: return -1;
    }
    return 0;
}

__global__ void reduce_partials_kernel(
    const float* __restrict__ partial,
    float* __restrict__ ey,
    size_t total_rows, int S, int n_ntiles, int nacc, int n_out)
{
    const size_t idx = (size_t)blockIdx.x * blockDim.x + threadIdx.x;
    if (idx >= total_rows) return;
    const size_t b = idx / S;
    const int s = (int)(idx % S);
    for (int o = 0; o < nacc; ++o) {
        float v = 0.0f;
        for (int nt = 0; nt < n_ntiles; ++nt)
            v += partial[(((size_t)b * n_ntiles + nt) * S + s) * nacc + o];
        ey[((size_t)b * S + s) * n_out + o] = v;
    }
}

template <int NOUT, int ACT>
static void launch_ft(
    const uint8_t* masksU, const float* diff, const float* base,
    const float* wbg, float* partial, float* ey, int B, int S, int M,
    int Mpad, int Npad, hipStream_t stream)
{
    constexpr int OIMG = (ACT == 3) ? 1 : NOUT;
    constexpr int NACC = NOUT;
    constexpr int KC = (OIMG >= 4) ? 8 : 16;
    const int n_ntiles = (Npad + 127) / 128;
    const int n_stiles = (S + S_TILE - 1) / S_TILE;
    dim3 grid(B * n_ntiles * n_stiles), block(256);
    size_t lds = (size_t)(2 * OIMG * KC * FT_NSTRIDE + OIMG * 128 + 128) * 4;
    fused_predict_tiled_kernel<NOUT, ACT><<<grid, block, lds, stream>>>(
        masksU, diff, base, wbg, partial, B, S, M, Mpad, Npad);
    size_t rows = (size_t)B * S;
    reduce_partials_kernel<<<dim3((unsigned)((rows + 255) / 256)), dim3(256),
                             0, stream>>>(
        partial, ey, rows, S, n_ntiles, NACC, NOUT);
}

template <int NOUT>
static void launch_ft_act(
    const uint8_t* masksU, const float* diff, const float* base,
    const float* wbg, float* partial, float* ey, int B, int S, int M,
    int Mpad, int Npad, int act, hipStream_t stream)
{
    switch (act) {
        case 0:
            launch_ft<NOUT, 0>(masksU, diff, base, wbg, partial, ey, B, S, M, Mpad, Npad, stream);
            break;
        case 1:
            launch_ft<NOUT, 1>(masksU, diff, base, wbg, partial, ey, B, S, M, Mpad, Npad, stream);
            break;
        case 3:
            if constexpr (NOUT == 2)
                launch_ft<NOUT, 3>(masksU, diff, base, wbg, partial, ey, B, S, M, Mpad, Npad, stream);
            break;
        default:
            launch_ft<NOUT, 2>(masksU, diff, base, wbg, partial, ey, B, S, M, Mpad, Npad, stream);
            break;
    }
}

extern "C" int launch_fused_predict_tiled(
    const uint8_t* masksU, const float* diff, const float* base,
    const float* wbg, float* partial, float* ey, int B, int S, int M,
    int Mpad, int Npad, int n_out, int act, hipStream_t stream)
{
    if (Npad % 16 != 0 || Mpad % 16 != 0) return -1;
    switch (n_out) {
        case 1: launch_ft_act<1>(masksU, diff, base, wbg, partial, ey, B, S, M, Mpad, Npad, act, stream); break;
        case 2: launch_ft_act<2>(masksU, diff, base, wbg, partial, ey, B, S, M, Mpad, Npad, act, stream); break;
        case 4: launch_ft_act<4>(masksU, diff, base, wbg, partial, ey, B, S, M, Mpad, Npad, act, stream); break;
        default: return -1;
    }
    return 0;
}


__global__ void fill_masks_packed_kernel(
    uint64_t* __restrict__ packed,
    const uint64_t* __restrict__ enum_packed,
    int B, int S, int M, int ne, int n_random,
    const float* __restrict__ cdf, const int* __restrict__ sizes, int n_sizes,
    int num_paired, uint32_t seed, const int32_t* __restrict__ inst_ids,
    int n_chunks)
{
    const int nblk = n_chunks / 8;
    const int b = blockIdx.x / nblk;
    const int cb = blockIdx.x % nblk;
    if (b >= B) return;
    uint64_t* prow = packed + (size_t)b * S;
    for (int i = cb * blockDim.x + threadIdx.x; i < ne; i += nblk * blockDim.x)
        prow[i] = enum_packed[i];

    const int lane = threadIdx.x & (WAVE - 1);
    const int chunk_id = cb * 8 + (threadIdx.x >> 6);
    const int chunk = (n_random + n_chunks - 1) / n_chunks;
    const int lo = chunk_id * chunk;
    const int hi = min(lo + chunk, n_random);
    if (lo >= hi) return;
    const uint64_t mmask = M >= 64 ? ~0ull : ((1ull << M) - 1ull);

    int remaining = hi - lo;
    int written = lo;
    uint32_t iter = 0;
    while (remaining > 0) {
        Philox rng;
        rng.init(seed, (uint32_t)inst_ids[b], iter,
                 (uint32_t)(chunk_id * WAVE + lane) | 0x52000000u);
        float u = (rng.next_u32() >> 8) * (1.0f / 16777216.0f);
        int si = 0;
        while (si < n_sizes - 1 && u > cdf[si]) ++si;
        int ssize = sizes[si];
        bool paired = ssize <= num_paired;

        uint64_t pairmask = __ballot(paired);
        uint64_t below = pairmask & ((1ull << lane) - 1ull);
        int rows_before = lane + __popcll(below);
        int total_rows = WAVE + __popcll(pairmask);

        if (rows_before < remaining) {
            uint64_t bits = 0ull;
            int got = 0;
            int guard = 0;
            while (got < ssize && guard < 65536) {
                uint32_t r = rng.next_below((uint32_t)M);
                uint64_t bit = 1ull << (r & 63);
                if (!(bits & bit)) { bits |= bit; ++got; }
                ++guard;
            }
            uint64_t* row = prow + ne + written + rows_before;
            row[0] = bits;
            if (paired && rows_before + 1 < remaining) row[1] = ~bits & mmask;
        }
        int consumed = total_rows < remaining ? total_rows : remaining;
        written += consumed;
        remaining -= consumed;
        ++iter;
    }
}

extern "C" int launch_fill_masks_packed(
    uint64_t* packed, const uint64_t* enum_packed, int B, int S, int M, int ne,
    int n_random, const float* cdf, const int* sizes, int n_sizes,
    int num_paired, uint32_t seed, const int32_t* inst_ids, hipStream_t stream)
{
    if (M < 1 || M > 64 || ne < 0 || n_random < 0 || ne + n_random != S)
        return -1;
    if (B <= 0 || S <= 0) return 0;
    const int n_chunks = kshap_sampler_chunks(n_random);
    fill_masks_packed_kernel<<<dim3(B * (n_chunks / 8)), dim3(8 * WAVE), 0,
                               stream>>>(
        packed, enum_packed, B, S, M, ne, n_random, cdf, sizes, n_sizes,
        num_paired, seed, inst_ids, n_chunks);
    return 0;
}

#define PREP_MAX_M 64
#define PREP_MAX_NOUT 8

__global__ __launch_bounds__(256)
void linear_prepare_kernel(
    const float* __restrict__ X,
    const float* __restrict__ W,
    const float* __restrict__ bias,
    const int64_t* __restrict__ col_group,
    const int64_t* __restrict__ vidx,
    const float* __restrict__ bgp,
    const double* __restrict__ lfnull64,
    float* __restrict__ diff,
    float* __restrict__ total,
    int D, int G, int N, int m, int Mpad, int Npad, int n_out, int OI,
    int act, int link)
{
    const int b = blockIdx.x;
    const int tid = threadIdx.x;
    const bool img3 = act == 3;
    if (img3) act = 2;
    __shared__ float xp_s[PREP_MAX_M * PREP_MAX_NOUT];
    __shared__ float xpi_s[PREP_MAX_M * PREP_MAX_NOUT];
    __shared__ int g_s[PREP_MAX_M];
    __shared__ double z_s[PREP_MAX_NOUT];
    const float* x = X + (size_t)b * D;

    if (tid < m) g_s[tid] = (int)vidx[tid];
    for (int p = tid; p < m * n_out; p += 256) {
        const int k = p / n_out, o = p % n_out;
        const int64_t g = vidx[k];
        const float* w = W + (size_t)o * D;
        float acc = 0.0f;
#pragma unroll 8
        for (int j = 0; j < D; ++j) {
            const float t = __fmul_rn(x[j], w[j]);
            acc = __fadd_rn(acc, col_group[j] == g ? t : 0.0f);
        }
        xp_s[p] = acc;
    }
    if (tid >= 256 - n_out) {
        const int o = tid - (256 - n_out);
        const float* w = W + (size_t)o * D;
        double z = (double)bias[o];
#pragma unroll 8
        for (int j = 0; j < D; ++j) z += (double)x[j] * (double)w[j];
        z_s[o] = z;
    }
    __syncthreads();
    for (int p = tid; p < m * OI; p += 256) {
        const int k = p / OI, oi = p % OI;
        xpi_s[p] = img3 ? __fsub_rn(xp_s[k * n_out + 1], xp_s[k * n_out])
                        : xp_s[k * n_out + oi];
    }
    if (tid < n_out) {
        const int o = tid;
        double p;
        if (act == 1) {
            p = 1.0 / (1.0 + exp(-z_s[o]));
        } else if (act == 2) {
            double mx = z_s[0];
            for (int q = 1; q < n_out; ++q) mx = fmax(mx, z_s[q]);
            double sum = 0.0;
            for (int q = 0; q < n_out; ++q) sum += exp(z_s[q] - mx);
            p = exp(z_s[o] - mx) / sum;
        } else {
            p = z_s[o];
        }
        if (link) {
            p = fmin(fmax(p, 1e-15), 1.0 - 1e-15);
            p = log(p / (1.0 - p));
        }
        total[(size_t)b * n_out + o] = (float)(p - lfnull64[o]);
    }
    __syncthreads();
    float* dout = diff + (size_t)b * OI * Mpad * Npad;
    const int per_img = Mpad * Npad;
    for (int idx = tid; idx < OI * per_img; idx += 256) {
        const int n = idx % Npad;
        const int k = (idx / Npad) % Mpad;
        const int oi = idx / per_img;
        float v = 0.0f;
        if (k < m && n < N && g_s[k] >= 0 && g_s[k] < G)
            v = __fsub_rn(xpi_s[k * OI + oi],
                          bgp[((size_t)n * G + g_s[k]) * OI + oi]);
        dout[idx] = v;
    }
}

extern "C" int launch_linear_prepare(
    const float* X, const float* W, const float* bias,
    const int64_t* col_group, const int64_t* vidx, const float* bgp,
    const double* lfnull64, float* diff, float* total, int B, int D, int G,
    int N, int m, int Mpad, int Npad, int n_out, int act, int link,
    hipStream_t stream)
{
    if (m < 1 || m > PREP_MAX_M || m > Mpad || N > Npad || n_out < 1
            || n_out > PREP_MAX_NOUT || act < 0 || act > 3)
        return -1;
    if (act == 3 && n_out != 2) return -1;
    const int OI = act == 3 ? 1 : n_out;
    if (B <= 0) return 0;
    linear_prepare_kernel<<<dim3(B), dim3(256), 0, stream>>>(
        X, W, bias, col_group, vidx, bgp, lfnull64, diff, total, D, G, N, m,
        Mpad, Npad, n_out, OI, act, link);
    return 0;
}


typedef __attribute__((ext_vector_type(4))) uint32_t u32x4;

__device__ __forceinline__ float dpp_add_quad1(float v) {
    return v + __builtin_bit_cast(float, __builtin_amdgcn_update_dpp(
        0, __builtin_bit_cast(int, v), 0xB1, 0xF, 0xF, true));
}
__device__ __forceinline__ float dpp_add_quad2(float v) {
    return v + __builtin_bit_cast(float, __builtin_amdgcn_update_dpp(
        0, __builtin_bit_cast(int, v), 0x4E, 0xF, 0xF, true));
}
__device__ __forceinline__ float dpp_add_half_mirror(float v) {
    return v + __builtin_bit_cast(float, __builtin_amdgcn_update_dpp(
        0, __builtin_bit_cast(int, v), 0x141, 0xF, 0xF, true));
}
__device__ __forceinline__ float dpp_add_mirror(float v) {
    return v + __builtin_bit_cast(float, __builtin_amdgcn_update_dpp(
        0, __builtin_bit_cast(int, v), 0x140, 0xF, 0xF, true));
}

template <int NOUT, int ACT, int NT, int KS, int MMA>
__global__ __launch_bounds__(256, 2)
void fused_predict_linear_packed_kernel(
    const uint64_t* __restrict__ packed,
    const float* __restrict__ diff,
    const float* __restrict__ base,
    const float* __restrict__ wbg,
    const float* __restrict__ lfnull,
    float* __restrict__ ey,
    int B, int S, int Mpad_rt, int link)
{
    constexpr int OIMG = (ACT == 3) ? 1 : NOUT;
    constexpr int NACC = (ACT == 3) ? 1 : NOUT;
    constexpr int NPAD = NT * 16;
    constexpr int NSTRIDE = NPAD + ((16 - (NPAD & 31)) & 31);
    constexpr bool SIG = (ACT == 1 || ACT == 3);
    constexpr bool SPL = (MMA == 1);
    static_assert(!SPL || (SIG && KS >= 1 && KS <= 3),
                  "split path: sigmoid-type activations, Mpad <= 12");
    constexpr bool BREG = SPL && (NT * OIMG <= 8);
    constexpr int NHALF = (NT * OIMG > 16) ? 2 : 1;
    constexpr int NTH = (NT + NHALF - 1) / NHALF;
    const int Mpad = KS > 0 ? KS * 4 : Mpad_rt;
    const int n_stiles = (S + S_TILE - 1) / S_TILE;
    const int b = blockIdx.x / n_stiles;
    const int stile = blockIdx.x % n_stiles;
    const int s0 = stile * S_TILE;
    const int tid = threadIdx.x;
    const int lane = tid & (WAVE - 1);
    const int wave = tid >> 6;

    extern __shared__ float lds[];
    float* diff_lds = lds;
    float* base_lds = diff_lds + OIMG * Mpad * NSTRIDE;
    float* wbg_lds = base_lds + OIMG * NPAD;
    u32x4* bw_lds = (u32x4*)lds;
    u32x4* bn_lds = bw_lds + OIMG * NT * 64;
    if constexpr (SPL) wbg_lds = (float*)(bn_lds + OIMG * NT * 64);

    const float scale = SIG ? -1.44269504088896340736f : 1.0f;
    const float* dsrc = diff + (size_t)b * OIMG * Mpad * NPAD;
    if constexpr (SPL) {
        for (int idx = tid; idx < OIMG * NT * 64; idx += 256) {
            const int l = idx & 63;
            const int o = (idx >> 6) / NT, ct = (idx >> 6) % NT;
            const int n = ct * 16 + (l & 15);
            const int q = l >> 4;
            uint32_t ph[3], pm[3], pl[3];
#pragma unroll
            for (int j = 0; j < 3; ++j) {
                const int g = 3 * q + j;
                const float v = g < KS * 4
                    ? __fmul_rn(dsrc[(o * (KS * 4) + g) * NPAD + n], scale) : 0.0f;
                const SplitBf16 sp = split_bf16(v);
                ph[j] = split_bf16_pattern(sp.hi);
                pm[j] = split_bf16_pattern(sp.mid);
                pl[j] = split_bf16_pattern(sp.lo);
            }
            const SplitBf16 sb = split_bf16(__fmul_rn(base[o * NPAD + n], scale));
            const uint32_t pb = q == 0 ? split_bf16_pattern(sb.hi)
                              : q == 1 ? split_bf16_pattern(sb.mid)
                              : q == 2 ? split_bf16_pattern(sb.lo) : 0u;
            bw_lds[idx] = (u32x4){ph[0] | (ph[1] << 16), ph[2] | (pm[0] << 16),
                                  pm[1] | (pm[2] << 16), pb};
            bn_lds[idx] = (u32x4){pl[0] | (pl[1] << 16), pl[2], 0u, 0u};
        }
    } else {
        for (int idx = tid; idx < OIMG * Mpad * NPAD; idx += 256) {
            int ok = idx / NPAD;
            int n = idx % NPAD;
            diff_lds[ok * NSTRIDE + n] = dsrc[idx] * scale;
        }
        for (int idx = tid; idx < OIMG * NPAD; idx += 256)
            base_lds[idx] = base[idx] * scale;
    }
    for (int idx = tid; idx < NPAD; idx += 256) wbg_lds[idx] = wbg[idx];
    __syncthreads();

    const int swave = wave * 16;
    const int arow = lane & 15;
    const int akcol = lane >> 4;
    const float* dbase = diff_lds + akcol * NSTRIDE + arow;
    const uint64_t* plane = packed + (size_t)b * S;

    bf16x8 bwr[BREG ? NT : 1][OIMG];
    bf16x8 bnr[BREG ? NT : 1][OIMG];
    if constexpr (BREG) {
#pragma unroll
        for (int ct = 0; ct < NT; ++ct)
#pragma unroll
            for (int o = 0; o < OIMG; ++o) {
                bwr[ct][o] = __builtin_bit_cast(bf16x8, bw_lds[(o * NT + ct) * 64 + lane]);
                bnr[ct][o] = __builtin_bit_cast(bf16x8, bn_lds[(o * NT + ct) * 64 + lane]);
            }
    }

    int srow = s0 + swave + arow;
    uint64_t bits_next = plane[min(srow, S - 1)];

    for (int sub = 0; sub < S_TILE / S_SUB; ++sub) {
        const int ssub0 = s0 + sub * S_SUB;
        if (ssub0 >= S) break;
        const uint64_t wv = srow < S ? bits_next : 0ull;
        const uint64_t w = wv >> akcol;
        srow += S_SUB;
        bits_next = plane[min(srow, S - 1)];

        float partial[NACC][4];
#pragma unroll
        for (int o = 0; o < NACC; ++o)
#pragma unroll
            for (int r = 0; r < 4; ++r) partial[o][r] = 0.0f;

#pragma unroll
        for (int half = 0; half < NHALF; ++half) {
        const int CT0 = half * NTH;
        const int CTN = half == 0 ? NTH : NT - NTH;

        f32x4 acc[NTH][OIMG];
#pragma unroll
        for (int ct = 0; ct < NTH; ++ct)
#pragma unroll
            for (int o = 0; o < OIMG; ++o) {
                if constexpr (!SPL) {
                    const float b0 =
                        ct < CTN ? base_lds[o * NPAD + (CT0 + ct) * 16 + arow] : 0.0f;
                    acc[ct][o] = (f32x4){b0, b0, b0, b0};
                }
            }

        if constexpr (SPL) {
            const uint32_t t = (uint32_t)(wv >> (3 * akcol));
            const uint32_t e0 = (t & 1u) ? 0x3F80u : 0u;
            const uint32_t e1 = (t & 2u) ? 0x3F80u : 0u;
            const uint32_t e2 = (t & 4u) ? 0x3F80u : 0u;
            const uint32_t e01 = e0 | (e1 << 16);
            const bf16x8 aw = __builtin_bit_cast(
                bf16x8, ((u32x4){e01, e2 | (e0 << 16), e1 | (e2 << 16), 0x3F80u}));
            const bf16x8 an = __builtin_bit_cast(
                bf16x8, ((u32x4){e01, e2, 0u, 0u}));
#pragma unroll
            for (int ct = 0; ct < NTH; ++ct) {
                if (ct < CTN) {
#pragma unroll
                    for (int o = 0; o < OIMG; ++o) {
                        bf16x8 bw;
                        if constexpr (BREG) bw = bwr[CT0 + ct][o];
                        else bw = __builtin_bit_cast(
                            bf16x8, bw_lds[(o * NT + CT0 + ct) * 64 + lane]);
                        acc[ct][o] = __builtin_amdgcn_mfma_f32_16x16x32_bf16(
                            aw, bw, (f32x4){0.0f, 0.0f, 0.0f, 0.0f}, 0, 0, 0);
                    }
                }
            }
#pragma unroll
            for (int ct = 0; ct < NTH; ++ct) {
                if (ct < CTN) {
#pragma unroll
                    for (int o = 0; o < OIMG; ++o) {
                        bf16x8 bn;
                        if constexpr (BREG) bn = bnr[CT0 + ct][o];
                        else bn = __builtin_bit_cast(
                            bf16x8, bn_lds[(o * NT + CT0 + ct) * 64 + lane]);
                        acc[ct][o] = __builtin_amdgcn_mfma_f32_16x16x32_bf16(
                            an, bn, acc[ct][o], 0, 0, 0);
                    }
                }
            }
        } else if constexpr (KS > 0) {
            const uint32_t wlo = (uint32_t)w;
#pragma unroll
            for (int ks = 0; ks < KS; ++ks) {
                const float a = (float)((wlo >> (4 * ks)) & 1u);
#pragma unroll
                for (int ct = 0; ct < NTH; ++ct) {
                    if (ct < CTN) {
#pragma unroll
                        for (int o = 0; o < OIMG; ++o) {
                            float bv = dbase[(o * (KS * 4) + ks * 4) * NSTRIDE + (CT0 + ct) * 16];
                            acc[ct][o] =
                                __builtin_amdgcn_mfma_f32_16x16x4f32(a, bv, acc[ct][o], 0, 0, 0);
                        }
                    }
                }
            }
        } else {
            uint64_t wk = w;
            for (int ks = 0; ks < Mpad; ks += 4) {
                const float a = (float)((uint32_t)wk & 1u);
                wk >>= 4;
#pragma unroll
                for (int ct = 0; ct < NTH; ++ct) {
                    if (ct < CTN) {
#pragma unroll
                        for (int o = 0; o < OIMG; ++o) {
                            float bv = dbase[(o * Mpad + ks) * NSTRIDE + (CT0 + ct) * 16];
                            acc[ct][o] =
                                __builtin_amdgcn_mfma_f32_16x16x4f32(a, bv, acc[ct][o], 0, 0, 0);
                        }
                    }
                }
            }
        }

#pragma unroll
        for (int ct = 0; ct < NTH; ++ct) {
            if (ct >= CTN) break;
            const float wn = wbg_lds[(CT0 + ct) * 16 + arow];
#pragma unroll
            for (int r = 0; r < 4; ++r) {
                float zz[NACC];
                if (SIG) {
#pragma unroll
                    for (int o = 0; o < NACC; ++o)
                        zz[o] = fast_rcp(1.0f + __builtin_amdgcn_exp2f(acc[ct][o][r]));
                } else if (ACT == 2 && NOUT == 2) {
                    float p1 = fast_rcp(1.0f + __expf(acc[ct][0][r] - acc[ct][1][r]));
                    zz[0] = 1.0f - p1;
                    zz[NACC - 1] = p1;
                } else if (ACT == 2) {
                    float mx = acc[ct][0][r];
#pragma unroll
                    for (int o = 1; o < NACC; ++o) mx = fmaxf(mx, acc[ct][o][r]);
                    float sum = 0.0f;
#pragma unroll
                    for (int o = 0; o < NACC; ++o) { zz[o] = __expf(acc[ct][o][r] - mx); sum += zz[o]; }
                    float inv = fast_rcp(sum);
#pragma unroll
                    for (int o = 0; o < NACC; ++o) zz[o] *= inv;
                } else {
#pragma unroll
                    for (int o = 0; o < NACC; ++o) zz[o] = acc[ct][o][r];
                }
#pragma unroll
                for (int o = 0; o < NACC; ++o) partial[o][r] += wn * zz[o];
            }
        }
        }

#pragma unroll
        for (int o = 0; o < NACC; ++o)
#pragma unroll
            for (int r = 0; r < 4; ++r) {
                float v = partial[o][r];
                v = dpp_add_quad1(v);
                v = dpp_add_quad2(v);
                v = dpp_add_half_mirror(v);
                v = dpp_add_mirror(v);
                partial[o][r] = v;
            }
        const int ss = ssub0 + swave + akcol * 4 + arow;
        if (arow < 4 && ss < S) {
            float out[NOUT];
            if (ACT == 3) {
                const float p1 = arow == 0 ? partial[0][0] : arow == 1 ? partial[0][1]
                               : arow == 2 ? partial[0][2] : partial[0][3];
                out[0] = 1.0f - p1;
                out[NOUT - 1] = p1;
            } else {
#pragma unroll
                for (int o = 0; o < NACC; ++o)
                    out[o] = arow == 0 ? partial[o][0] : arow == 1 ? partial[o][1]
                           : arow == 2 ? partial[o][2] : partial[o][3];
            }
            if (link == 1) {
#pragma unroll
                for (int o = 0; o < NOUT; ++o) {
                    const float p = fminf(fmaxf(out[o], 1e-7f), 0.9999999f);
                    out[o] = 0.69314718055994530942f
                        * (__builtin_amdgcn_logf(p) - __builtin_amdgcn_logf(1.0f - p));
                }
            }
            if (lfnull != nullptr) {
#pragma unroll
                for (int o = 0; o < NOUT; ++o) out[o] -= lfnull[o];
            }
            float* dst = ey + ((size_t)b * S + ss) * NOUT;
            if constexpr (NOUT == 2) {
                *(float2*)dst = make_float2(out[0], out[1]);
            } else if constexpr (NOUT == 4) {
                *(float4*)dst = make_float4(out[0], out[1], out[2], out[3]);
            } else {
                dst[0] = out[0];
            }
        }
    }
}

template <int NOUT, int ACT, int NT>
static int launch_fpp_ks(
    const uint64_t* packed, const float* diff, const float* base,
    const float* wbg, const float* lfnull, float* ey, int B, int S, int Mpad,
    int link, int mma, hipStream_t stream)
{
    const int n_stiles = (S + S_TILE - 1) / S_TILE;
    dim3 grid(B * n_stiles), block(256);
    constexpr int NPAD = NT * 16;
    constexpr int NSTRIDE = NPAD + ((16 - (NPAD & 31)) & 31);
    constexpr int OIMG = (ACT == 3) ? 1 : NOUT;
    size_t lds = (size_t)(OIMG * Mpad * NSTRIDE + OIMG * NPAD + NPAD) * 4;
    if (lds > 64 * 1024) return -1;
#define KSHAP_FPP(KSV, MMAV) \
    fused_predict_linear_packed_kernel<NOUT, ACT, NT, KSV, MMAV> \
        <<<grid, block, lds, stream>>>(packed, diff, base, wbg, lfnull, ey, \
                                       B, S, Mpad, link)
    if constexpr (ACT == 1 || ACT == 3) {
        const size_t lds_split = (size_t)OIMG * NT * 64 * 32 + (size_t)NPAD * 4;
        if (mma != 0 && Mpad <= 12 && lds_split <= 64 * 1024) {
            lds = lds_split;
            switch (Mpad / 4) {
                case 1: KSHAP_FPP(1, 1); return 0;
                case 2: KSHAP_FPP(2, 1); return 0;
                case 3: KSHAP_FPP(3, 1); return 0;
                default: break;
            }
        }
        switch (Mpad / 4) {
            case 1: KSHAP_FPP(1, 0); return 0;
            case 2: KSHAP_FPP(2, 0); return 0;
            case 3: KSHAP_FPP(3, 0); return 0;
            case 4: KSHAP_FPP(4, 0); return 0;
            default: break;
        }
    }
    KSHAP_FPP(0, 0);
#undef KSHAP_FPP
    return 0;
}

template <int NOUT, int ACT>
static int launch_fpp_nt(
    const uint64_t* packed, const float* diff, const float* base,
    const float* wbg, const float* lfnull, float* ey, int B, int S, int Mpad,
    int Npad, int link, int mma, hipStream_t stream)
{
#define KSHAP_FPP_NT(NTV) \
    case NTV: \
        return launch_fpp_ks<NOUT, ACT, NTV>(packed, diff, base, wbg, lfnull, \
                                             ey, B, S, Mpad, link, mma, stream);
    switch (Npad / 16) {
        KSHAP_FPP_NT(1) KSHAP_FPP_NT(2) KSHAP_FPP_NT(3) KSHAP_FPP_NT(4)
        KSHAP_FPP_NT(5) KSHAP_FPP_NT(6) KSHAP_FPP_NT(7) KSHAP_FPP_NT(8)
    }
#undef KSHAP_FPP_NT
    return -1;
}

template <int NOUT>
static int launch_fpp_act(
    const uint64_t* packed, const float* diff, const float* base,
    const float* wbg, const float* lfnull, float* ey, int B, int S, int Mpad,
    int Npad, int act, int link, int mma, hipStream_t stream)
{
    switch (act) {
        case 0:
            return launch_fpp_nt<NOUT, 0>(packed, diff, base, wbg, lfnull, ey, B, S, Mpad, Npad, link, mma, stream);
        case 1:
            return launch_fpp_nt<NOUT, 1>(packed, diff, base, wbg, lfnull, ey, B, S, Mpad, Npad, link, mma, stream);
        case 2:
            return launch_fpp_nt<NOUT, 2>(packed, diff, base, wbg, lfnull, ey, B, S, Mpad, Npad, link, mma, stream);
        case 3:
            if constexpr (NOUT == 2)
                return launch_fpp_nt<NOUT, 3>(packed, diff, base, wbg, lfnull, ey, B, S, Mpad, Npad, link, mma, stream);
            return -1;
        default:
            return -1;
    }
}

extern "C" int launch_fused_predict_linear_packed(
    const uint64_t* packed, const float* diff, const float* base,
    const float* wbg, const float* lfnull, float* ey, int B, int S, int Mpad,
    int Npad, int n_out, int act, int link, hipStream_t stream, int mma)
{
    if (Mpad < 4 || Mpad > MAX_MPAD || Mpad % 4 != 0 || Npad % 16 != 0
            || Npad < 16 || Npad / 16 > 8 || mma < -1 || mma > 1)
        return -1;
    if (link != 0 && (link != 1 || lfnull == nullptr)) return -1;
    if (B <= 0 || S <= 0) return 0;
    switch (n_out) {
        case 1: return launch_fpp_act<1>(packed, diff, base, wbg, lfnull, ey, B, S, Mpad, Npad, act, link, mma, stream);
        case 2: return launch_fpp_act<2>(packed, diff, base, wbg, lfnull, ey, B, S, Mpad, Npad, act, link, mma, stream);
        case 4: return launch_fpp_act<4>(packed, diff, base, wbg, lfnull, ey, B, S, Mpad, Npad, act, link, mma, stream);
        default: return -1;
    }
}

template <int J>
__device__ __forceinline__ float dpp_row_bcast(float v) {
    return __builtin_bit_cast(float, __builtin_amdgcn_update_dpp(
        0, __builtin_bit_cast(int, v), 0x150 + J, 0xF, 0xF, true));
}
template <int J>
__device__ __forceinline__ uint32_t dpp_row_bcast_u(uint32_t v) {
    return (uint32_t)__builtin_amdgcn_update_dpp(0, (int)v, 0x150 + J, 0xF, 0xF, true);
}

template <int I, int N, class F>
__device__ __forceinline__ void static_for(F&& f) {
    if constexpr (I < N) {
        f(std::integral_constant<int, I>{});
        static_for<I + 1, N>(f);
    }
}

#define WLSP_MAXM 15

template <int NOUT>
struct WlsSample {
    uint32_t bits;
    float w;
    float e[NOUT];
    bool ok;
};

template <int NOUT>
__global__ __launch_bounds__(64)
void wls_solve_packed_kernel(
    const uint64_t* __restrict__ packed,
    const float* __restrict__ kw,
    const float* __restrict__ ey_adj,
    const float* __restrict__ total,
    const int64_t* __restrict__ vidx,
    float* __restrict__ phi_full,
    int B, int S, int M, int n_out, int G)
{
    const int b = blockIdx.x;
    if (b >= B) return;
    const int lane = threadIdx.x;
    const int arow = lane & 15;
    const int akk = lane >> 4;
    const int mm = M - 1;

    __shared__ float As[16][17];
    __shared__ float phi_s[16][NOUT];
    __shared__ int g_s[16];

    float tot[NOUT];
#pragma unroll
    for (int o = 0; o < NOUT; ++o)
        tot[o] = o < n_out ? total[(size_t)b * n_out + o] : 0.0f;
    if (lane < M) g_s[lane] = (int)vidx[lane];

    const uint64_t* pbase = packed + (size_t)b * S;
    const float* eyb = ey_adj + (size_t)b * S * n_out;
    const int slot = 4 * arow + akk;
    const bool is_a = arow < mm;
    const int osel = arow - mm;

    auto load = [&](int base) __attribute__((always_inline)) {
        WlsSample<NOUT> s;
        s.ok = base + slot < S;
        const int idx = min(base + slot, S - 1);
        s.bits = (uint32_t)pbase[idx];
        s.w = kw[idx];
#pragma unroll
        for (int o = 0; o < NOUT; ++o)
            s.e[o] = eyb[(size_t)idx * n_out + min(o, n_out - 1)];
        return s;
    };

    auto gram_block = [&](f32x4& acc, const WlsSample<NOUT>& raw, int rem) __attribute__((always_inline)) {
        WlsSample<NOUT> s;
        s.bits = raw.ok ? raw.bits : 0u;
        s.w = raw.ok ? raw.w : 0.0f;
        const float ml = (float)((s.bits >> mm) & 1u);
        float wey[NOUT];
#pragma unroll
        for (int o = 0; o < NOUT; ++o)
            wey[o] = o < n_out ? s.w * (raw.e[o] - ml * tot[o]) : 0.0f;
        static_for<0, 16>([&](auto jc) __attribute__((always_inline)) {
            constexpr int j = decltype(jc)::value;
            if (4 * j < rem) {
                const uint32_t bb = dpp_row_bcast_u<j>(s.bits);
                const float ww = dpp_row_bcast<j>(s.w);
                float es = 0.0f;
#pragma unroll
                for (int o = 0; o < NOUT; ++o) {
                    const float t = dpp_row_bcast<j>(wey[o]);
                    es = (osel == o) ? t : es;
                }
                const float d = (float)((int)((bb >> arow) & 1u)
                                        - (int)((bb >> mm) & 1u));
                const float a = is_a ? d : 0.0f;
                const float bv = is_a ? ww * d : es;
                acc = __builtin_amdgcn_mfma_f32_16x16x4f32(a, bv, acc, 0, 0, 0);
            }
        });
    };

    f32x4 acc[4];
#pragma unroll
    for (int w = 0; w < 4; ++w) acc[w] = (f32x4){0, 0, 0, 0};

    WlsSample<NOUT> cur = load(0);
    for (int c0 = 0; c0 < S; c0 += WLS_CHUNK) {
        static_for<0, 4>([&](auto wc) __attribute__((always_inline)) {
            constexpr int w = decltype(wc)::value;
            const int base = c0 + w * 64;
            if (base < S) {
                const WlsSample<NOUT> nxt = load(base + 64);
                gram_block(acc[w], cur, S - base);
                cur = nxt;
            }
        });
    }
#pragma unroll
    for (int r = 0; r < 4; ++r)
        As[akk * 4 + r][arow] = ((acc[0][r] + acc[1][r]) + acc[2][r]) + acc[3][r];
    __syncthreads();

    float L[WLSP_MAXM];
#pragma unroll
    for (int c = 0; c < WLSP_MAXM; ++c) {
        const float v = As[arow][c];
        L[c] = (arow < mm && c < mm) ? v : (arow == c ? 1.0f : 0.0f);
    }
    static_for<0, WLSP_MAXM>([&](auto kc) __attribute__((always_inline)) {
        constexpr int k = decltype(kc)::value;
        const float d = sqrtf(fmaxf(dpp_row_bcast<k>(L[k]), 1e-20f));
        const float inv = 1.0f / d;
        const float lk = L[k] * inv;
        L[k] = (arow == k) ? d : lk;
        static_for<k + 1, WLSP_MAXM>([&](auto cc) __attribute__((always_inline)) {
            constexpr int c = decltype(cc)::value;
            L[c] = fmaf(-lk, dpp_row_bcast<c>(lk), L[c]);
        });
    });

#pragma unroll 1
    for (int o0 = 0; o0 < NOUT; o0 += 4) {
        const int o = o0 + akk;
        const bool live = o < n_out;
        const float r_own = (live && arow < mm) ? As[arow][mm + (live ? o : 0)] : 0.0f;
        float y[WLSP_MAXM], wv[WLSP_MAXM];
        static_for<0, WLSP_MAXM>([&](auto ic) __attribute__((always_inline)) {
            constexpr int i = decltype(ic)::value;
            float v = dpp_row_bcast<i>(r_own);
            static_for<0, i>([&](auto tc) __attribute__((always_inline)) {
                constexpr int t = decltype(tc)::value;
                v = fmaf(-dpp_row_bcast<i>(L[t]), y[t], v);
            });
            y[i] = v / dpp_row_bcast<i>(L[i]);
        });
        static_for<0, WLSP_MAXM>([&](auto ic) __attribute__((always_inline)) {
            constexpr int i = WLSP_MAXM - 1 - decltype(ic)::value;
            float v = y[i];
            static_for<i + 1, WLSP_MAXM>([&](auto tc) __attribute__((always_inline)) {
                constexpr int t = decltype(tc)::value;
                v = fmaf(-dpp_row_bcast<t>(L[i]), wv[t], v);
            });
            wv[i] = v / dpp_row_bcast<i>(L[i]);
        });
        float sumw = 0.0f;
#pragma unroll
        for (int i = 0; i < WLSP_MAXM; ++i) sumw += wv[i];
        if (live) {
            float mine = 0.0f;
#pragma unroll
            for (int i = 0; i < WLSP_MAXM; ++i) mine = (arow == i) ? wv[i] : mine;
            float to = 0.0f;
#pragma unroll
            for (int oo = 0; oo < NOUT; ++oo) to = (o == oo) ? tot[oo] : to;
            if (arow < mm) phi_s[arow][o] = mine;
            if (arow == mm) phi_s[mm][o] = to - sumw;
        }
    }
    __syncthreads();
    float* prow = phi_full + (size_t)b * G * n_out;
    for (int idx = lane; idx < G * n_out; idx += 64) {
        const int g = idx / n_out, o = idx % n_out;
        float v = 0.0f;
        for (int k = 0; k < M; ++k)
            if (g_s[k] == g) v = phi_s[k][o];
        prow[idx] = v;
    }
}

extern "C" int launch_wls_solve_packed(
    const uint64_t* packed, const float* kw, const float* ey_adj,
    const float* total, const int64_t* vidx, float* phi_full, int B, int S,
    int M, int n_out, int G, hipStream_t stream)
{
    if (M < 2 || M > G || n_out < 1 || n_out > WLS_MAX_NOUT
            || (M - 1) + n_out > 16)
        return -1;
    if (B <= 0) return 0;
#define KSHAP_WLSP(NO) \
    wls_solve_packed_kernel<NO><<<dim3(B), dim3(64), 0, stream>>>( \
        packed, kw, ey_adj, total, vidx, phi_full, B, S, M, n_out, G)
    if (n_out == 1) KSHAP_WLSP(1);
    else if (n_out == 2) KSHAP_WLSP(2);
    else if (n_out <= 4) KSHAP_WLSP(4);
    else KSHAP_WLSP(8);
#undef KSHAP_WLSP
    return 0;
}


__global__ __launch_bounds__(256)
void varying_keys_kernel(
    const float* __restrict__ X,
    const float* __restrict__ bg_min,
    const float* __restrict__ bg_max,
    const float* __restrict__ tol_min,
    const float* __restrict__ tol_max,
    const int64_t* __restrict__ col_group,
    int64_t* __restrict__ keys,
    int B, int D)
{
    const int lane = threadIdx.x & (WAVE - 1);
    const int b = blockIdx.x * (blockDim.x / WAVE) + (threadIdx.x >> 6);
    if (b >= B) return;
    const float* xr = X + (size_t)b * D;
    uint64_t bits = 0ull;
    for (int j = lane; j < D; j += WAVE) {
        const float x = xr[j];
        const bool cmin = fabsf(__fsub_rn(bg_min[j], x)) <= tol_min[j];
        const bool cmax = fabsf(__fsub_rn(bg_max[j], x)) <= tol_max[j];
        const int64_t g = col_group[j];
        if (!(cmin && cmax) && g >= 0 && g < 64) bits |= 1ull << g;
    }
    uint32_t lo = (uint32_t)bits, hi = (uint32_t)(bits >> 32);
#pragma unroll
    for (int off = 1; off < WAVE; off <<= 1) {
        lo |= (uint32_t)__shfl_xor((int)lo, off, WAVE);
        hi |= (uint32_t)__shfl_xor((int)hi, off, WAVE);
    }
    if (lane == 0) keys[b] = (int64_t)(((uint64_t)hi << 32) | lo);
}

__global__ __launch_bounds__(1024)
void varying_probe_reduce_kernel(
    const int64_t* __restrict__ keys,
    int64_t* __restrict__ probe,
    int B)
{
    const int64_t k0 = keys[0];
    int differs = 0;
    for (int i = threadIdx.x; i < B; i += blockDim.x)
        differs |= (keys[i] != k0);
    differs = __syncthreads_or(differs);
    if (threadIdx.x == 0) {
        probe[0] = differs ? 0 : 1;
        probe[1] = k0;
    }
}

extern "C" int launch_varying_probe(
    const float* X, const float* bg_min, const float* bg_max,
    const float* tol_min, const float* tol_max, const int64_t* col_group,
    int64_t* keys, int64_t* probe, int B, int D, int G, hipStream_t stream)
{
    if (B < 1 || D < 1 || G < 1 || G > 62) return -1;
    const int wpb = 256 / WAVE;
    varying_keys_kernel<<<dim3((B + wpb - 1) / wpb), dim3(256), 0, stream>>>(
        X, bg_min, bg_max, tol_min, tol_max, col_group, keys, B, D);
    varying_probe_reduce_kernel<<<dim3(1), dim3(1024), 0, stream>>>(
        keys, probe, B);
    return 0;
}
```

Measured before the change: 6.523 million explanations/s.

## Fuse packed linear predict and WLS solve into one kernel with ey in LDS

Adds a kernel that runs the split-bf16 MFMA predict for one instance per block, keeps the per-sample expected outputs in shared memory, then builds the Gram matrix and solves the WLS system in the same block. This removes the global ey buffer write and read-back and one kernel launch. The trade-off is one 256-thread block per instance with LDS capped at 52 KiB, which limits S and occupancy and may leave the GPU underused compared with the separate wide predict kernel. It is gated by a new packed_fuse config switch with an auto default and shape checks.

```diff
diff --git a/distributedkernelshap_amd/config.py b/distributedkernelshap_amd/config.py
--- a/distributedkernelshap_amd/config.py
+++ b/distributedkernelshap_amd/config.py
@@ -61,10 +61,24 @@
     fused_predict: bool = True
     predict_dtype: str = "fp32"
     packed_mma: str = "auto"
+    packed_fuse: str = "auto"
     synth_chunk_rows: int = 1 << 21
     l1_device: bool = True
     module_autocast: str = "off"
     module_channels_last: bool = True
+
+    PACKED_FUSE_MODES = ("auto", "on", "off")
+
+    def __post_init__(self):
+        self.check_packed_fuse()
+
+    def check_packed_fuse(self) -> str:
+        if self.packed_fuse not in self.PACKED_FUSE_MODES:
+            raise ValueError(
+                "packed_fuse must be 'auto', 'on' or 'off', "
+                f"got {self.packed_fuse!r}"
+            )
+        return self.packed_fuse
 
 
 @dataclass
diff --git a/distributedkernelshap_amd/ops/gpu_engine.py b/distributedkernelshap_amd/ops/gpu_engine.py
--- a/distributedkernelshap_amd/ops/gpu_engine.py
+++ b/distributedkernelshap_amd/ops/gpu_engine.py
@@ -916,6 +916,17 @@
                 f"packed_mma must be 'auto', 'f32' or 'split', got {mode!r}"
             ) from None
 
+    def _packed_fuse_ok(self, m, mpad, s, c) -> bool:
+        mode = self.engine.kernels.check_packed_fuse()
+        if mode == "off" or self._packed_mma() == 0:
+            return False
+        return (
+            mpad <= 12
+            and (m - 1) + self.n_out <= 16
+            and 1 <= s <= self.ext.predict_solve_max_s(
+                c["npad"], self.n_out, c["act"])
+        )
+
     def _packed_pipeline(self, X_dev, plan, vidx_t, ids_dev, phi_full,
                          timer=None):
         t = self.torch
@@ -937,6 +948,15 @@
             X_dev, self.linear["W"], self.linear["b"], self.col_group, vidx_t,
             c["bgp"], c["lfnull64"], diff, total, c["act"], c["link"],
         )
+        if self._packed_fuse_ok(m, mpad, s, c):
+            self.ext.predict_solve_linear_packed(
+                packed, diff, c["base"], c["wbg"], kw, total, vidx_t, phi_full,
+                c["act"], c["link"], c["lfnull"],
+            )
+            if timer is not None:
+                timer.mark("predict")
+                timer.mark("wls")
+            return
         ey = self._buf("ey", (b, s, self.n_out))
         self.ext.fused_predict_linear_packed(
             packed, diff, c["base"], c["wbg"], ey, c["act"], c["link"],
diff --git a/distributedkernelshap_amd/ops/hip/bindings.cpp b/distributedkernelshap_amd/ops/hip/bindings.cpp
--- a/distributedkernelshap_amd/ops/hip/bindings.cpp
+++ b/distributedkernelshap_amd/ops/hip/bindings.cpp
@@ -86,6 +86,15 @@
     const uint64_t* packed, const float* kw, const float* ey_adj,
     const float* total, const int64_t* vidx, float* phi_full, int B, int S,
     int M, int n_out, int G, hipStream_t stream);
+
+extern "C" int launch_predict_solve_linear_packed(
+    const uint64_t* packed, const float* diff, const float* base,
+    const float* wbg, const float* lfnull, const float* kw, const float* total,
+    const int64_t* vidx, float* phi_full, float* ey_out, int B, int S,
+    int Mpad, int Npad, int M, int n_out, int G, int act, int link,
+    hipStream_t stream);
+
+extern "C" int predict_solve_linear_packed_max_s(int Npad, int n_out, int act);
 
 extern "C" int launch_varying_probe(
     const float* X, const float* bg_min, const float* bg_max,
@@ -344,6 +353,63 @@
         G, current_stream());
     TORCH_CHECK(rc == 0, "wls_solve_packed: unsupported shape (2<=M<=G, "
                          "(M-1)+n_out<=16)");
+}
+
+int64_t predict_solve_max_s(int64_t npad, int64_t n_out, int64_t act) {
+    return predict_solve_linear_packed_max_s((int)npad, (int)n_out, (int)act);
+}
+
+void predict_solve_linear_packed(
+    torch::Tensor packed, torch::Tensor diff, torch::Tensor base,
+    torch::Tensor wbg, torch::Tensor kw, torch::Tensor total,
+    torch::Tensor vidx, torch::Tensor phi_full, int64_t act, int64_t link,
+    c10::optional<torch::Tensor> lfnull, c10::optional<torch::Tensor> ey_out) {
+    CHECK_DEV(packed); CHECK_DEV(diff); CHECK_DEV(base); CHECK_DEV(wbg);
+    CHECK_DEV(kw); CHECK_DEV(total); CHECK_DEV(vidx); CHECK_DEV(phi_full);
+    CHECK_I64(packed); CHECK_F32(diff); CHECK_F32(base); CHECK_F32(wbg);
+    CHECK_F32(kw); CHECK_F32(total); CHECK_I64(vidx); CHECK_F32(phi_full);
+    TORCH_CHECK(packed.dim() == 2 && diff.dim() == 4 && base.dim() == 2
+                && phi_full.dim() == 3 && vidx.dim() == 1 && total.dim() == 2,
+                "operand ranks");
+    int B = packed.size(0), S = packed.size(1), M = vidx.size(0);
+    int Mpad = diff.size(2), Npad = diff.size(3);
+    int n_out = phi_full.size(2), G = phi_full.size(1);
+    int oimg = (act == 3) ? 1 : n_out;
+    TORCH_CHECK(diff.size(0) == B && diff.size(1) == oimg, "diff (B,oimg,Mpad,Npad) vs act");
+    TORCH_CHECK(base.size(0) == oimg && base.size(1) == Npad, "base shape");
+    TORCH_CHECK(wbg.numel() == Npad, "wbg shape");
+    TORCH_CHECK(kw.numel() == S, "kw must be (S,)");
+    TORCH_CHECK(total.size(0) == B && total.size(1) == n_out, "total shape");
+    TORCH_CHECK(phi_full.size(0) == B, "phi_full shape");
+    const float* lf = nullptr;
+    if (lfnull.has_value()) {
+        CHECK_DEV(lfnull.value()); CHECK_F32(lfnull.value());
+        TORCH_CHECK(lfnull->numel() == n_out, "lfnull must be (n_out,)");
+        lf = lfnull->data_ptr<float>();
+    }
+    TORCH_CHECK(link == 0 || (link == 1 && lf != nullptr),
+                "link must be 0, or 1 with lfnull given");
+    float* eyp = nullptr;
+    if (ey_out.has_value()) {
+        CHECK_DEV(ey_out.value()); CHECK_F32(ey_out.value());
+        TORCH_CHECK(ey_out->dim() == 3 && ey_out->size(0) == B
+                    && ey_out->size(1) == S && ey_out->size(2) == n_out,
+                    "ey_out must be (B,S,n_out)");
+        eyp = ey_out->data_ptr<float>();
+    }
+    int rc = launch_predict_solve_linear_packed(
+        reinterpret_cast<const uint64_t*>(packed.data_ptr<int64_t>()),
+        diff.data_ptr<float>(), base.data_ptr<float>(), wbg.data_ptr<float>(),
+        lf, kw.data_ptr<float>(), total.data_ptr<float>(),
+        vidx.data_ptr<int64_t>(), phi_full.data_ptr<float>(), eyp, B, S, Mpad,
+        Npad, M, n_out, G, (int)act, (int)link, current_stream());
+    TORCH_CHECK(rc == 0, "predict_solve_linear_packed: unsupported shape (act "
+                         "1 or 3, Mpad in {4,8,12}, Npad%16==0, (Npad/16)*"
+                         "images<=16, n_out in {1,2,4}, 2<=M<=min(G,Mpad), "
+                         "(M-1)+n_out<=16, S>=1, and the block's LDS with "
+                         "S*n_out*4 bytes of ey within PSL_LDS_CAP = 52 KiB, "
+                         "which keeps three blocks on a CU: see "
+                         "predict_solve_max_s)");
 }
 
 void varying_probe(
@@ -840,6 +906,19 @@
           pybind11::arg("packed"), pybind11::arg("kw"), pybind11::arg("ey_adj"),
           pybind11::arg("total"), pybind11::arg("vidx"),
           pybind11::arg("phi_full"));
+    m.def("predict_solve_linear_packed", &predict_solve_linear_packed,
+          "K3p (split-operand path) and K7p in one kernel, one block per "
+          "instance, ey kept in LDS; raises for shapes outside its reach. "
+          "ey_out (B,S,n_out), when given, also receives the adjusted ey",
+          pybind11::arg("packed"), pybind11::arg("diff"), pybind11::arg("base"),
+          pybind11::arg("wbg"), pybind11::arg("kw"), pybind11::arg("total"),
+          pybind11::arg("vidx"), pybind11::arg("phi_full"), pybind11::arg("act"),
+          pybind11::arg("link"), pybind11::arg("lfnull"),
+          pybind11::arg("ey_out") = pybind11::none());
+    m.def("predict_solve_max_s", &predict_solve_max_s,
+          "largest S predict_solve_linear_packed takes at (npad, n_out, act); "
+          "0 when the shape is outside its reach at any S",
+          pybind11::arg("npad"), pybind11::arg("n_out"), pybind11::arg("act"));
     m.def("varying_probe", &varying_probe,
           "varying-pattern probe (K1p): per-instance group bit keys and "
           "[all(keys == keys[0]), keys[0]] in two launches, no host sync",
diff --git a/distributedkernelshap_amd/ops/hip/kshap_kernels.hip b/distributedkernelshap_amd/ops/hip/kshap_kernels.hip
--- a/distributedkernelshap_amd/ops/hip/kshap_kernels.hip
+++ b/distributedkernelshap_amd/ops/hip/kshap_kernels.hip
@@ -2116,6 +2116,243 @@
         0, __builtin_bit_cast(int, v), 0x140, 0xF, 0xF, true));
 }
 
+template <int OIMG, int NT, int KS>
+__device__ __forceinline__ void fpp_stage_split(
+    const float* __restrict__ dsrc, const float* __restrict__ base,
+    const float scale, u32x4* bw_lds, u32x4* bn_lds, const int tid)
+{
+    constexpr int NPAD = NT * 16;
+    for (int idx = tid; idx < OIMG * NT * 64; idx += 256) {
+        const int l = idx & 63;
+        const int o = (idx >> 6) / NT, ct = (idx >> 6) % NT;
+        const int n = ct * 16 + (l & 15);
+        const int q = l >> 4;
+        uint32_t ph[3], pm[3], pl[3];
+#pragma unroll
+        for (int j = 0; j < 3; ++j) {
+            const int g = 3 * q + j;
+            const float v = g < KS * 4
+                ? __fmul_rn(dsrc[(o * (KS * 4) + g) * NPAD + n], scale) : 0.0f;
+            const SplitBf16 sp = split_bf16(v);
+            ph[j] = split_bf16_pattern(sp.hi);
+            pm[j] = split_bf16_pattern(sp.mid);
+            pl[j] = split_bf16_pattern(sp.lo);
+        }
+        const SplitBf16 sb = split_bf16(__fmul_rn(base[o * NPAD + n], scale));
+        const uint32_t pb = q == 0 ? split_bf16_pattern(sb.hi)
+                          : q == 1 ? split_bf16_pattern(sb.mid)
+                          : q == 2 ? split_bf16_pattern(sb.lo) : 0u;
+        bw_lds[idx] = (u32x4){ph[0] | (ph[1] << 16), ph[2] | (pm[0] << 16),
+                              pm[1] | (pm[2] << 16), pb};
+        bn_lds[idx] = (u32x4){pl[0] | (pl[1] << 16), pl[2], 0u, 0u};
+    }
+}
+
+template <int NOUT, int ACT, int NT, int KS, int MMA, class Frag, class Store>
+__device__ __forceinline__ void fpp_subtile(
+    const uint64_t wv, const int lane, const int Mpad,
+    const Frag& bwr, const Frag& bnr,
+    const u32x4* bw_lds, const u32x4* bn_lds,
+    const float* dbase, const float* base_lds, const float* wbg_lds,
+    const int link, const float* __restrict__ lfnull, const bool row_ok,
+    Store&& store)
+{
+    constexpr int OIMG = (ACT == 3) ? 1 : NOUT;
+    constexpr int NACC = (ACT == 3) ? 1 : NOUT;
+    constexpr int NPAD = NT * 16;
+    constexpr int NSTRIDE = NPAD + ((16 - (NPAD & 31)) & 31);
+    constexpr bool SIG = (ACT == 1 || ACT == 3);
+    constexpr bool SPL = (MMA == 1);
+    constexpr bool BREG = SPL && (NT * OIMG <= 8);
+    constexpr int NHALF = (NT * OIMG > 16) ? 2 : 1;
+    constexpr int NTH = (NT + NHALF - 1) / NHALF;
+    const int arow = lane & 15;
+    const int akcol = lane >> 4;
+    const uint64_t w = wv >> akcol;
+
+    float partial[NACC][4];
+#pragma unroll
+    for (int o = 0; o < NACC; ++o)
+#pragma unroll
+        for (int r = 0; r < 4; ++r) partial[o][r] = 0.0f;
+
+#pragma unroll
+    for (int half = 0; half < NHALF; ++half) {
+    const int CT0 = half * NTH;
+    const int CTN = half == 0 ? NTH : NT - NTH;
+
+    f32x4 acc[NTH][OIMG];
+#pragma unroll
+    for (int ct = 0; ct < NTH; ++ct)
+#pragma unroll
+        for (int o = 0; o < OIMG; ++o) {
+            if constexpr (!SPL) {
+                const float b0 =
+                    ct < CTN ? base_lds[o * NPAD + (CT0 + ct) * 16 + arow] : 0.0f;
+                acc[ct][o] = (f32x4){b0, b0, b0, b0};
+            }
+        }
+
+    if constexpr (SPL) {
+        const uint32_t t = (uint32_t)(wv >> (3 * akcol));
+        const uint32_t e0 = (t & 1u) ? 0x3F80u : 0u;
+        const uint32_t e1 = (t & 2u) ? 0x3F80u : 0u;
+        const uint32_t e2 = (t & 4u) ? 0x3F80u : 0u;
+        const uint32_t e01 = e0 | (e1 << 16);
+        const bf16x8 aw = __builtin_bit_cast(
+            bf16x8, ((u32x4){e01, e2 | (e0 << 16), e1 | (e2 << 16), 0x3F80u}));
+        const bf16x8 an = __builtin_bit_cast(
+            bf16x8, ((u32x4){e01, e2, 0u, 0u}));
+#pragma unroll
+        for (int ct = 0; ct < NTH; ++ct) {
+            if (ct < CTN) {
+#pragma unroll
+                for (int o = 0; o < OIMG; ++o) {
+                    bf16x8 bw;
+                    if constexpr (BREG) bw = bwr[CT0 + ct][o];
+                    else bw = __builtin_bit_cast(
+                        bf16x8, bw_lds[(o * NT + CT0 + ct) * 64 + lane]);
+                    acc[ct][o] = __builtin_amdgcn_mfma_f32_16x16x32_bf16(
+                        aw, bw, (f32x4){0.0f, 0.0f, 0.0f, 0.0f}, 0, 0, 0);
+                }
+            }
+        }
+#pragma unroll
+        for (int ct = 0; ct < NTH; ++ct) {
+            if (ct < CTN) {
+#pragma unroll
+                for (int o = 0; o < OIMG; ++o) {
+                    bf16x8 bn;
+                    if constexpr (BREG) bn = bnr[CT0 + ct][o];
+                    else bn = __builtin_bit_cast(
+                        bf16x8, bn_lds[(o * NT + CT0 + ct) * 64 + lane]);
+                    acc[ct][o] = __builtin_amdgcn_mfma_f32_16x16x32_bf16(
+                        an, bn, acc[ct][o], 0, 0, 0);
+                }
+            }
+        }
+    } else if constexpr (KS > 0) {
+        const uint32_t wlo = (uint32_t)w;
+#pragma unroll
+        for (int ks = 0; ks < KS; ++ks) {
+            const float a = (float)((wlo >> (4 * ks)) & 1u);
+#pragma unroll
+            for (int ct = 0; ct < NTH; ++ct) {
+                if (ct < CTN) {
+#pragma unroll
+                    for (int o = 0; o < OIMG; ++o) {
+                        float bv = dbase[(o * (KS * 4) + ks * 4) * NSTRIDE + (CT0 + ct) * 16];
+                        acc[ct][o] =
+                            __builtin_amdgcn_mfma_f32_16x16x4f32(a, bv, acc[ct][o], 0, 0, 0);
+                    }
+                }
+            }
+        }
+    } else {
+        uint64_t wk = w;
+        for (int ks = 0; ks < Mpad; ks += 4) {
+            const float a = (float)((uint32_t)wk & 1u);
+            wk >>= 4;
+#pragma unroll
+            for (int ct = 0; ct < NTH; ++ct) {
+                if (ct < CTN) {
+#pragma unroll
+                    for (int o = 0; o < OIMG; ++o) {
+                        float bv = dbase[(o * Mpad + ks) * NSTRIDE + (CT0 + ct) * 16];
+                        acc[ct][o] =
+                            __builtin_amdgcn_mfma_f32_16x16x4f32(a, bv, acc[ct][o], 0, 0, 0);
+                    }
+                }
+            }
+        }
+    }
+
+#pragma unroll
+    for (int ct = 0; ct < NTH; ++ct) {
+        if (ct >= CTN) break;
+        const float wn = wbg_lds[(CT0 + ct) * 16 + arow];
+#pragma unroll
+        for (int r = 0; r < 4; ++r) {
+            float zz[NACC];
+            if (SIG) {
+#pragma unroll
+                for (int o = 0; o < NACC; ++o)
+                    zz[o] = fast_rcp(1.0f + __builtin_amdgcn_exp2f(acc[ct][o][r]));
+            } else if (ACT == 2 && NOUT == 2) {
+                float p1 = fast_rcp(1.0f + __expf(acc[ct][0][r] - acc[ct][1][r]));
+                zz[0] = 1.0f - p1;
+                zz[NACC - 1] = p1;
+            } else if (ACT == 2) {
+                float mx = acc[ct][0][r];
+#pragma unroll
+                for (int o = 1; o < NACC; ++o) mx = fmaxf(mx, acc[ct][o][r]);
+                float sum = 0.0f;
+#pragma unroll
+                for (int o = 0; o < NACC; ++o) { zz[o] = __expf(acc[ct][o][r] - mx); sum += zz[o]; }
+                float inv = fast_rcp(sum);
+#pragma unroll
+                for (int o = 0; o < NACC; ++o) zz[o] *= inv;
+            } else {
+#pragma unroll
+                for (int o = 0; o < NACC; ++o) zz[o] = acc[ct][o][r];
+            }
+#pragma unroll
+            for (int o = 0; o < NACC; ++o) partial[o][r] += wn * zz[o];
+        }
+    }
+    }
+
+#pragma unroll
+    for (int o = 0; o < NACC; ++o)
+#pragma unroll
+        for (int r = 0; r < 4; ++r) {
+            float v = partial[o][r];
+            v = dpp_add_quad1(v);
+            v = dpp_add_quad2(v);
+            v = dpp_add_half_mirror(v);
+            v = dpp_add_mirror(v);
+            partial[o][r] = v;
+        }
+    if (arow < 4 && row_ok) {
+        float out[NOUT];
+        if (ACT == 3) {
+            const float p1 = arow == 0 ? partial[0][0] : arow == 1 ? partial[0][1]
+                           : arow == 2 ? partial[0][2] : partial[0][3];
+            out[0] = 1.0f - p1;
+            out[NOUT - 1] = p1;
+        } else {
+#pragma unroll
+            for (int o = 0; o < NACC; ++o)
+                out[o] = arow == 0 ? partial[o][0] : arow == 1 ? partial[o][1]
+                       : arow == 2 ? partial[o][2] : partial[o][3];
+        }
+        if (link == 1) {
+#pragma unroll
+            for (int o = 0; o < NOUT; ++o) {
+                const float p = fminf(fmaxf(out[o], 1e-7f), 0.9999999f);
+                out[o] = 0.69314718055994530942f
+                    * (__builtin_amdgcn_logf(p) - __builtin_amdgcn_logf(1.0f - p));
+            }
+        }
+        if (lfnull != nullptr) {
+#pragma unroll
+            for (int o = 0; o < NOUT; ++o) out[o] -= lfnull[o];
+        }
+        store(out);
+    }
+}
+
+template <int NOUT>
+__device__ __forceinline__ void store_ey_row(float* dst, const float (&out)[NOUT]) {
+    if constexpr (NOUT == 2) {
+        *(float2*)dst = make_float2(out[0], out[1]);
+    } else if constexpr (NOUT == 4) {
+        *(float4*)dst = make_float4(out[0], out[1], out[2], out[3]);
+    } else {
+        dst[0] = out[0];
+    }
+}
+
 template <int NOUT, int ACT, int NT, int KS, int MMA>
 __global__ __launch_bounds__(256, 2)
 void fused_predict_linear_packed_kernel(
@@ -2128,7 +2365,6 @@
     int B, int S, int Mpad_rt, int link)
 {
     constexpr int OIMG = (ACT == 3) ? 1 : NOUT;
-    constexpr int NACC = (ACT == 3) ? 1 : NOUT;
     constexpr int NPAD = NT * 16;
     constexpr int NSTRIDE = NPAD + ((16 - (NPAD & 31)) & 31);
     constexpr bool SIG = (ACT == 1 || ACT == 3);
@@ -2136,8 +2372,6 @@
     static_assert(!SPL || (SIG && KS >= 1 && KS <= 3),
                   "split path: sigmoid-type activations, Mpad <= 12");
     constexpr bool BREG = SPL && (NT * OIMG <= 8);
-    constexpr int NHALF = (NT * OIMG > 16) ? 2 : 1;
-    constexpr int NTH = (NT + NHALF - 1) / NHALF;
     const int Mpad = KS > 0 ? KS * 4 : Mpad_rt;
     const int n_stiles = (S + S_TILE - 1) / S_TILE;
     const int b = blockIdx.x / n_stiles;
@@ -2158,30 +2392,7 @@
     const float scale = SIG ? -1.44269504088896340736f : 1.0f;
     const float* dsrc = diff + (size_t)b * OIMG * Mpad * NPAD;
     if constexpr (SPL) {
-        for (int idx = tid; idx < OIMG * NT * 64; idx += 256) {
-            const int l = idx & 63;
-            const int o = (idx >> 6) / NT, ct = (idx >> 6) % NT;
-            const int n = ct * 16 + (l & 15);
-            const int q = l >> 4;
-            uint32_t ph[3], pm[3], pl[3];
-#pragma unroll
-            for (int j = 0; j < 3; ++j) {
-                const int g = 3 * q + j;
-                const float v = g < KS * 4
-                    ? __fmul_rn(dsrc[(o * (KS * 4) + g) * NPAD + n], scale) : 0.0f;
-                const SplitBf16 sp = split_bf16(v);
-                ph[j] = split_bf16_pattern(sp.hi);
-                pm[j] = split_bf16_pattern(sp.mid);
-                pl[j] = split_bf16_pattern(sp.lo);
-            }
-            const SplitBf16 sb = split_bf16(__fmul_rn(base[o * NPAD + n], scale));
-            const uint32_t pb = q == 0 ? split_bf16_pattern(sb.hi)
-                              : q == 1 ? split_bf16_pattern(sb.mid)
-                              : q == 2 ? split_bf16_pattern(sb.lo) : 0u;
-            bw_lds[idx] = (u32x4){ph[0] | (ph[1] << 16), ph[2] | (pm[0] << 16),
-                                  pm[1] | (pm[2] << 16), pb};
-            bn_lds[idx] = (u32x4){pl[0] | (pl[1] << 16), pl[2], 0u, 0u};
-        }
+        fpp_stage_split<OIMG, NT, KS>(dsrc, base, scale, bw_lds, bn_lds, tid);
     } else {
         for (int idx = tid; idx < OIMG * Mpad * NPAD; idx += 256) {
             int ok = idx / NPAD;
@@ -2219,188 +2430,16 @@
         const int ssub0 = s0 + sub * S_SUB;
         if (ssub0 >= S) break;
         const uint64_t wv = srow < S ? bits_next : 0ull;
-        const uint64_t w = wv >> akcol;
         srow += S_SUB;
         bits_next = plane[min(srow, S - 1)];
 
-        float partial[NACC][4];
-#pragma unroll
-        for (int o = 0; o < NACC; ++o)
-#pragma unroll
-            for (int r = 0; r < 4; ++r) partial[o][r] = 0.0f;
-
-#pragma unroll
-        for (int half = 0; half < NHALF; ++half) {
-        const int CT0 = half * NTH;
-        const int CTN = half == 0 ? NTH : NT - NTH;
-
-        f32x4 acc[NTH][OIMG];
-#pragma unroll
-        for (int ct = 0; ct < NTH; ++ct)
-#pragma unroll
-            for (int o = 0; o < OIMG; ++o) {
-                if constexpr (!SPL) {
-                    const float b0 =
-                        ct < CTN ? base_lds[o * NPAD + (CT0 + ct) * 16 + arow] : 0.0f;
-                    acc[ct][o] = (f32x4){b0, b0, b0, b0};
-                }
-            }
-
-        if constexpr (SPL) {
-            const uint32_t t = (uint32_t)(wv >> (3 * akcol));
-            const uint32_t e0 = (t & 1u) ? 0x3F80u : 0u;
-            const uint32_t e1 = (t & 2u) ? 0x3F80u : 0u;
-            const uint32_t e2 = (t & 4u) ? 0x3F80u : 0u;
-            const uint32_t e01 = e0 | (e1 << 16);
-            const bf16x8 aw = __builtin_bit_cast(
-                bf16x8, ((u32x4){e01, e2 | (e0 << 16), e1 | (e2 << 16), 0x3F80u}));
-            const bf16x8 an = __builtin_bit_cast(
-                bf16x8, ((u32x4){e01, e2, 0u, 0u}));
-#pragma unroll
-            for (int ct = 0; ct < NTH; ++ct) {
-                if (ct < CTN) {
-#pragma unroll
-                    for (int o = 0; o < OIMG; ++o) {
-                        bf16x8 bw;
-                        if constexpr (BREG) bw = bwr[CT0 + ct][o];
-                        else bw = __builtin_bit_cast(
-                            bf16x8, bw_lds[(o * NT + CT0 + ct) * 64 + lane]);
-                        acc[ct][o] = __builtin_amdgcn_mfma_f32_16x16x32_bf16(
-                            aw, bw, (f32x4){0.0f, 0.0f, 0.0f, 0.0f}, 0, 0, 0);
-                    }
-                }
-            }
-#pragma unroll
-            for (int ct = 0; ct < NTH; ++ct) {
-                if (ct < CTN) {
-#pragma unroll
-                    for (int o = 0; o < OIMG; ++o) {
-                        bf16x8 bn;
-                        if constexpr (BREG) bn = bnr[CT0 + ct][o];
-                        else bn = __builtin_bit_cast(
-                            bf16x8, bn_lds[(o * NT + CT0 + ct) * 64 + lane]);
-                        acc[ct][o] = __builtin_amdgcn_mfma_f32_16x16x32_bf16(
-                            an, bn, acc[ct][o], 0, 0, 0);
-                    }
-                }
-            }
-        } else if constexpr (KS > 0) {
-            const uint32_t wlo = (uint32_t)w;
-#pragma unroll
-            for (int ks = 0; ks < KS; ++ks) {
-                const float a = (float)((wlo >> (4 * ks)) & 1u);
-#pragma unroll
-                for (int ct = 0; ct < NTH; ++ct) {
-                    if (ct < CTN) {
-#pragma unroll
-                        for (int o = 0; o < OIMG; ++o) {
-                            float bv = dbase[(o * (KS * 4) + ks * 4) * NSTRIDE + (CT0 + ct) * 16];
-                            acc[ct][o] =
-                                __builtin_amdgcn_mfma_f32_16x16x4f32(a, bv, acc[ct][o], 0, 0, 0);
-                        }
-                    }
-                }
-            }
-        } else {
-            uint64_t wk = w;
-            for (int ks = 0; ks < Mpad; ks += 4) {
-                const float a = (float)((uint32_t)wk & 1u);
-                wk >>= 4;
-#pragma unroll
-                for (int ct = 0; ct < NTH; ++ct) {
-                    if (ct < CTN) {
-#pragma unroll
-                        for (int o = 0; o < OIMG; ++o) {
-                            float bv = dbase[(o * Mpad + ks) * NSTRIDE + (CT0 + ct) * 16];
-                            acc[ct][o] =
-                                __builtin_amdgcn_mfma_f32_16x16x4f32(a, bv, acc[ct][o], 0, 0, 0);
-                        }
-                    }
-                }
-            }
-        }
-
-#pragma unroll
-        for (int ct = 0; ct < NTH; ++ct) {
-            if (ct >= CTN) break;
-            const float wn = wbg_lds[(CT0 + ct) * 16 + arow];
-#pragma unroll
-            for (int r = 0; r < 4; ++r) {
-                float zz[NACC];
-                if (SIG) {
-#pragma unroll
-                    for (int o = 0; o < NACC; ++o)
-                        zz[o] = fast_rcp(1.0f + __builtin_amdgcn_exp2f(acc[ct][o][r]));
-                } else if (ACT == 2 && NOUT == 2) {
-                    float p1 = fast_rcp(1.0f + __expf(acc[ct][0][r] - acc[ct][1][r]));
-                    zz[0] = 1.0f - p1;
-                    zz[NACC - 1] = p1;
-                } else if (ACT == 2) {
-                    float mx = acc[ct][0][r];
-#pragma unroll
-                    for (int o = 1; o < NACC; ++o) mx = fmaxf(mx, acc[ct][o][r]);
-                    float sum = 0.0f;
-#pragma unroll
-                    for (int o = 0; o < NACC; ++o) { zz[o] = __expf(acc[ct][o][r] - mx); sum += zz[o]; }
-                    float inv = fast_rcp(sum);
-#pragma unroll
-                    for (int o = 0; o < NACC; ++o) zz[o] *= inv;
-                } else {
-#pragma unroll
-                    for (int o = 0; o < NACC; ++o) zz[o] = acc[ct][o][r];
-                }
-#pragma unroll
-                for (int o = 0; o < NACC; ++o) partial[o][r] += wn * zz[o];
-            }
-        }
-        }
-
-#pragma unroll
-        for (int o = 0; o < NACC; ++o)
-#pragma unroll
-            for (int r = 0; r < 4; ++r) {
-                float v = partial[o][r];
-                v = dpp_add_quad1(v);
-                v = dpp_add_quad2(v);
-                v = dpp_add_half_mirror(v);
-                v = dpp_add_mirror(v);
-                partial[o][r] = v;
-            }
         const int ss = ssub0 + swave + akcol * 4 + arow;
-        if (arow < 4 && ss < S) {
-            float out[NOUT];
-            if (ACT == 3) {
-                const float p1 = arow == 0 ? partial[0][0] : arow == 1 ? partial[0][1]
-                               : arow == 2 ? partial[0][2] : partial[0][3];
-                out[0] = 1.0f - p1;
-                out[NOUT - 1] = p1;
-            } else {
-#pragma unroll
-                for (int o = 0; o < NACC; ++o)
-                    out[o] = arow == 0 ? partial[o][0] : arow == 1 ? partial[o][1]
-                           : arow == 2 ? partial[o][2] : partial[o][3];
-            }
-            if (link == 1) {
-#pragma unroll
-                for (int o = 0; o < NOUT; ++o) {
-                    const float p = fminf(fmaxf(out[o], 1e-7f), 0.9999999f);
-                    out[o] = 0.69314718055994530942f
-                        * (__builtin_amdgcn_logf(p) - __builtin_amdgcn_logf(1.0f - p));
-                }
-            }
-            if (lfnull != nullptr) {
-#pragma unroll
-                for (int o = 0; o < NOUT; ++o) out[o] -= lfnull[o];
-            }
-            float* dst = ey + ((size_t)b * S + ss) * NOUT;
-            if constexpr (NOUT == 2) {
-                *(float2*)dst = make_float2(out[0], out[1]);
-            } else if constexpr (NOUT == 4) {
-                *(float4*)dst = make_float4(out[0], out[1], out[2], out[3]);
-            } else {
-                dst[0] = out[0];
-            }
-        }
+        fpp_subtile<NOUT, ACT, NT, KS, MMA>(
+            wv, lane, Mpad, bwr, bnr, bw_lds, bn_lds, dbase, base_lds, wbg_lds,
+            link, lfnull, ss < S,
+            [&](const float (&out)[NOUT]) __attribute__((always_inline)) {
+                store_ey_row<NOUT>(ey + ((size_t)b * S + ss) * NOUT, out);
+            });
     }
 }
 
@@ -2531,102 +2570,49 @@
     bool ok;
 };
 
+
 template <int NOUT>
-__global__ __launch_bounds__(64)
-void wls_solve_packed_kernel(
-    const uint64_t* __restrict__ packed,
-    const float* __restrict__ kw,
-    const float* __restrict__ ey_adj,
-    const float* __restrict__ total,
-    const int64_t* __restrict__ vidx,
-    float* __restrict__ phi_full,
-    int B, int S, int M, int n_out, int G)
-{
-    const int b = blockIdx.x;
-    if (b >= B) return;
-    const int lane = threadIdx.x;
+__device__ __forceinline__ void wls_gram_block(
+    f32x4& acc, const WlsSample<NOUT>& raw, const int rem, const int mm,
+    const int n_out, const float (&tot)[NOUT], const int arow)
+{
+    const bool is_a = arow < mm;
+    const int osel = arow - mm;
+    WlsSample<NOUT> s;
+    s.bits = raw.ok ? raw.bits : 0u;
+    s.w = raw.ok ? raw.w : 0.0f;
+    const float ml = (float)((s.bits >> mm) & 1u);
+    float wey[NOUT];
+#pragma unroll
+    for (int o = 0; o < NOUT; ++o)
+        wey[o] = o < n_out ? s.w * (raw.e[o] - ml * tot[o]) : 0.0f;
+    static_for<0, 16>([&](auto jc) __attribute__((always_inline)) {
+        constexpr int j = decltype(jc)::value;
+        if (4 * j < rem) {
+            const uint32_t bb = dpp_row_bcast_u<j>(s.bits);
+            const float ww = dpp_row_bcast<j>(s.w);
+            float es = 0.0f;
+#pragma unroll
+            for (int o = 0; o < NOUT; ++o) {
+                const float t = dpp_row_bcast<j>(wey[o]);
+                es = (osel == o) ? t : es;
+            }
+            const float d = (float)((int)((bb >> arow) & 1u)
+                                    - (int)((bb >> mm) & 1u));
+            const float a = is_a ? d : 0.0f;
+            const float bv = is_a ? ww * d : es;
+            acc = __builtin_amdgcn_mfma_f32_16x16x4f32(a, bv, acc, 0, 0, 0);
+        }
+    });
+}
+
+template <int NOUT>
+__device__ __forceinline__ void wls_factor_solve(
+    const float (*As)[17], float (*phi_s)[NOUT], const float (&tot)[NOUT],
+    const int lane, const int mm, const int n_out)
+{
     const int arow = lane & 15;
     const int akk = lane >> 4;
-    const int mm = M - 1;
-
-    __shared__ float As[16][17];
-    __shared__ float phi_s[16][NOUT];
-    __shared__ int g_s[16];
-
-    float tot[NOUT];
-#pragma unroll
-    for (int o = 0; o < NOUT; ++o)
-        tot[o] = o < n_out ? total[(size_t)b * n_out + o] : 0.0f;
-    if (lane < M) g_s[lane] = (int)vidx[lane];
-
-    const uint64_t* pbase = packed + (size_t)b * S;
-    const float* eyb = ey_adj + (size_t)b * S * n_out;
-    const int slot = 4 * arow + akk;
-    const bool is_a = arow < mm;
-    const int osel = arow - mm;
-
-    auto load = [&](int base) __attribute__((always_inline)) {
-        WlsSample<NOUT> s;
-        s.ok = base + slot < S;
-        const int idx = min(base + slot, S - 1);
-        s.bits = (uint32_t)pbase[idx];
-        s.w = kw[idx];
-#pragma unroll
-        for (int o = 0; o < NOUT; ++o)
-            s.e[o] = eyb[(size_t)idx * n_out + min(o, n_out - 1)];
-        return s;
-    };
-
-    auto gram_block = [&](f32x4& acc, const WlsSample<NOUT>& raw, int rem) __attribute__((always_inline)) {
-        WlsSample<NOUT> s;
-        s.bits = raw.ok ? raw.bits : 0u;
-        s.w = raw.ok ? raw.w : 0.0f;
-        const float ml = (float)((s.bits >> mm) & 1u);
-        float wey[NOUT];
-#pragma unroll
-        for (int o = 0; o < NOUT; ++o)
-            wey[o] = o < n_out ? s.w * (raw.e[o] - ml * tot[o]) : 0.0f;
-        static_for<0, 16>([&](auto jc) __attribute__((always_inline)) {
-            constexpr int j = decltype(jc)::value;
-            if (4 * j < rem) {
-                const uint32_t bb = dpp_row_bcast_u<j>(s.bits);
-                const float ww = dpp_row_bcast<j>(s.w);
-                float es = 0.0f;
-#pragma unroll
-                for (int o = 0; o < NOUT; ++o) {
-                    const float t = dpp_row_bcast<j>(wey[o]);
-                    es = (osel == o) ? t : es;
-                }
-                const float d = (float)((int)((bb >> arow) & 1u)
-                                        - (int)((bb >> mm) & 1u));
-                const float a = is_a ? d : 0.0f;
-                const float bv = is_a ? ww * d : es;
-                acc = __builtin_amdgcn_mfma_f32_16x16x4f32(a, bv, acc, 0, 0, 0);
-            }
-        });
-    };
-
-    f32x4 acc[4];
-#pragma unroll
-    for (int w = 0; w < 4; ++w) acc[w] = (f32x4){0, 0, 0, 0};
-
-    WlsSample<NOUT> cur = load(0);
-    for (int c0 = 0; c0 < S; c0 += WLS_CHUNK) {
-        static_for<0, 4>([&](auto wc) __attribute__((always_inline)) {
-            constexpr int w = decltype(wc)::value;
-            const int base = c0 + w * 64;
-            if (base < S) {
-                const WlsSample<NOUT> nxt = load(base + 64);
-                gram_block(acc[w], cur, S - base);
-                cur = nxt;
-            }
-        });
-    }
-#pragma unroll
-    for (int r = 0; r < 4; ++r)
-        As[akk * 4 + r][arow] = ((acc[0][r] + acc[1][r]) + acc[2][r]) + acc[3][r];
-    __syncthreads();
-
     float L[WLSP_MAXM];
 #pragma unroll
     for (int c = 0; c < WLSP_MAXM; ++c) {
@@ -2683,8 +2669,13 @@
             if (arow == mm) phi_s[mm][o] = to - sumw;
         }
     }
-    __syncthreads();
-    float* prow = phi_full + (size_t)b * G * n_out;
+}
+
+template <int NOUT>
+__device__ __forceinline__ void wls_scatter(
+    const float (*phi_s)[NOUT], const int* g_s, float* __restrict__ prow,
+    const int lane, const int M, const int n_out, const int G)
+{
     for (int idx = lane; idx < G * n_out; idx += 64) {
         const int g = idx / n_out, o = idx % n_out;
         float v = 0.0f;
@@ -2692,6 +2683,77 @@
             if (g_s[k] == g) v = phi_s[k][o];
         prow[idx] = v;
     }
+}
+
+template <int NOUT>
+__global__ __launch_bounds__(64)
+void wls_solve_packed_kernel(
+    const uint64_t* __restrict__ packed,
+    const float* __restrict__ kw,
+    const float* __restrict__ ey_adj,
+    const float* __restrict__ total,
+    const int64_t* __restrict__ vidx,
+    float* __restrict__ phi_full,
+    int B, int S, int M, int n_out, int G)
+{
+    const int b = blockIdx.x;
+    if (b >= B) return;
+    const int lane = threadIdx.x;
+    const int arow = lane & 15;
+    const int akk = lane >> 4;
+    const int mm = M - 1;
+
+    __shared__ float As[16][17];
+    __shared__ float phi_s[16][NOUT];
+    __shared__ int g_s[16];
+
+    float tot[NOUT];
+#pragma unroll
+    for (int o = 0; o < NOUT; ++o)
+        tot[o] = o < n_out ? total[(size_t)b * n_out + o] : 0.0f;
+    if (lane < M) g_s[lane] = (int)vidx[lane];
+
+    const uint64_t* pbase = packed + (size_t)b * S;
+    const float* eyb = ey_adj + (size_t)b * S * n_out;
+    const int slot = 4 * arow + akk;
+
+    auto load = [&](int base) __attribute__((always_inline)) {
+        WlsSample<NOUT> s;
+        s.ok = base + slot < S;
+        const int idx = min(base + slot, S - 1);
+        s.bits = (uint32_t)pbase[idx];
+        s.w = kw[idx];
+#pragma unroll
+        for (int o = 0; o < NOUT; ++o)
+            s.e[o] = eyb[(size_t)idx * n_out + min(o, n_out - 1)];
+        return s;
+    };
+
+    f32x4 acc[4];
+#pragma unroll
+    for (int w = 0; w < 4; ++w) acc[w] = (f32x4){0, 0, 0, 0};
+
+    WlsSample<NOUT> cur = load(0);
+    for (int c0 = 0; c0 < S; c0 += WLS_CHUNK) {
+        static_for<0, 4>([&](auto wc) __attribute__((always_inline)) {
+            constexpr int w = decltype(wc)::value;
+            const int base = c0 + w * 64;
+            if (base < S) {
+                const WlsSample<NOUT> nxt = load(base + 64);
+                wls_gram_block<NOUT>(acc[w], cur, S - base, mm, n_out, tot, arow);
+                cur = nxt;
+            }
+        });
+    }
+#pragma unroll
+    for (int r = 0; r < 4; ++r)
+        As[akk * 4 + r][arow] = ((acc[0][r] + acc[1][r]) + acc[2][r]) + acc[3][r];
+    __syncthreads();
+
+    wls_factor_solve<NOUT>(As, phi_s, tot, lane, mm, n_out);
+    __syncthreads();
+    wls_scatter<NOUT>(phi_s, g_s, phi_full + (size_t)b * G * n_out, lane, M,
+                      n_out, G);
 }
 
 extern "C" int launch_wls_solve_packed(
@@ -2714,6 +2776,226 @@
     return 0;
 }
 
+#define PSL_LDS_CAP (52 * 1024)
+#define PSL_MAX_TILES 16
+
+static constexpr int psl_fixed_lds(int oimg, int nt, int nout) {
+    return oimg * nt * 64 * 32 + nt * 16 * 4 + 4 * 16 * 17 * 4 + 16 * 17 * 4
+           + 16 * nout * 4 + 16 * 4;
+}
+
+template <int NOUT, int ACT, int NT, int KS>
+__global__ __launch_bounds__(256, 3)
+void predict_solve_linear_packed_kernel(
+    const uint64_t* __restrict__ packed,
+    const float* __restrict__ diff,
+    const float* __restrict__ base,
+    const float* __restrict__ wbg,
+    const float* __restrict__ lfnull,
+    const float* __restrict__ kw,
+    const float* __restrict__ total,
+    const int64_t* __restrict__ vidx,
+    float* __restrict__ phi_full,
+    float* __restrict__ ey_out,
+    int B, int S, int M, int G, int link)
+{
+    constexpr int OIMG = (ACT == 3) ? 1 : NOUT;
+    constexpr int NPAD = NT * 16;
+    static_assert((ACT == 1 || ACT == 3) && KS >= 1 && KS <= 3
+                  && NT * OIMG <= PSL_MAX_TILES, "split path, one column half");
+    constexpr bool BREG = NT * OIMG <= 8;
+    const int b = blockIdx.x;
+    const int tid = threadIdx.x;
+    const int lane = tid & (WAVE - 1);
+    const int wave = tid >> 6;
+    const int arow = lane & 15;
+    const int akcol = lane >> 4;
+    const int mm = M - 1;
+
+    extern __shared__ float lds[];
+    u32x4* bw_lds = (u32x4*)lds;
+    u32x4* bn_lds = bw_lds + OIMG * NT * 64;
+    float* wbg_lds = (float*)(bn_lds + OIMG * NT * 64);
+    float (*acc_s)[16][17] = (float (*)[16][17])(wbg_lds + NPAD);
+    float (*As)[17] = (float (*)[17])(acc_s + 4);
+    float (*phi_s)[NOUT] = (float (*)[NOUT])(As + 16);
+    int* g_s = (int*)(phi_s + 16);
+    float* ey_s = (float*)(g_s + 16);
+
+    fpp_stage_split<OIMG, NT, KS>(
+        diff + (size_t)b * OIMG * (KS * 4) * NPAD, base,
+        -1.44269504088896340736f, bw_lds, bn_lds, tid);
+    for (int idx = tid; idx < NPAD; idx += 256) wbg_lds[idx] = wbg[idx];
+    if (tid < M) g_s[tid] = (int)vidx[tid];
+    __syncthreads();
+
+    const uint64_t* plane = packed + (size_t)b * S;
+    {
+        bf16x8 bwr[BREG ? NT : 1][OIMG];
+        bf16x8 bnr[BREG ? NT : 1][OIMG];
+        if constexpr (BREG) {
+#pragma unroll
+            for (int ct = 0; ct < NT; ++ct)
+#pragma unroll
+                for (int o = 0; o < OIMG; ++o) {
+                    bwr[ct][o] = __builtin_bit_cast(bf16x8, bw_lds[(o * NT + ct) * 64 + lane]);
+                    bnr[ct][o] = __builtin_bit_cast(bf16x8, bn_lds[(o * NT + ct) * 64 + lane]);
+                }
+        }
+
+        const int swave = wave * 16;
+        int srow = swave + arow;
+        uint64_t bits_next = plane[min(srow, S - 1)];
+        for (int ssub0 = 0; ssub0 < S; ssub0 += S_SUB) {
+            const uint64_t wv = srow < S ? bits_next : 0ull;
+            srow += S_SUB;
+            bits_next = plane[min(srow, S - 1)];
+
+            const int ss = ssub0 + swave + akcol * 4 + arow;
+            fpp_subtile<NOUT, ACT, NT, KS, 1>(
+                wv, lane, KS * 4, bwr, bnr, bw_lds, bn_lds, nullptr, nullptr,
+                wbg_lds, link, lfnull, ss < S,
+                [&](const float (&out)[NOUT]) __attribute__((always_inline)) {
+                    store_ey_row<NOUT>(ey_s + (size_t)ss * NOUT, out);
+                    if (ey_out != nullptr)
+                        store_ey_row<NOUT>(ey_out + ((size_t)b * S + ss) * NOUT, out);
+                });
+        }
+    }
+    __syncthreads();
+
+    float tot[NOUT];
+#pragma unroll
+    for (int o = 0; o < NOUT; ++o) tot[o] = total[(size_t)b * NOUT + o];
+    const int slot = 4 * arow + akcol;
+    auto load = [&](int base) __attribute__((always_inline)) {
+        WlsSample<NOUT> s;
+        s.ok = base + slot < S;
+        const int idx = min(base + slot, S - 1);
+        s.bits = (uint32_t)plane[idx];
+        s.w = kw[idx];
+#pragma unroll
+        for (int o = 0; o < NOUT; ++o) s.e[o] = ey_s[idx * NOUT + o];
+        return s;
+    };
+    f32x4 acc = (f32x4){0, 0, 0, 0};
+    WlsSample<NOUT> cur = load(wave * 64);
+    for (int base = wave * 64; base < S; base += WLS_CHUNK) {
+        const WlsSample<NOUT> nxt = load(base + WLS_CHUNK);
+        wls_gram_block<NOUT>(acc, cur, S - base, mm, NOUT, tot, arow);
+        cur = nxt;
+    }
+#pragma unroll
+    for (int r = 0; r < 4; ++r) acc_s[wave][akcol * 4 + r][arow] = acc[r];
+    __syncthreads();
+    if (wave == 0) {
+#pragma unroll
+        for (int r = 0; r < 4; ++r) {
+            const int i = akcol * 4 + r;
+            As[i][arow] = ((acc_s[0][i][arow] + acc_s[1][i][arow])
+                           + acc_s[2][i][arow]) + acc_s[3][i][arow];
+        }
+    }
+    __syncthreads();
+
+    if (wave == 0) wls_factor_solve<NOUT>(As, phi_s, tot, lane, mm, NOUT);
+    __syncthreads();
+    if (wave == 0)
+        wls_scatter<NOUT>(phi_s, g_s, phi_full + (size_t)b * G * NOUT, lane, M,
+                          NOUT, G);
+}
+
+extern "C" int predict_solve_linear_packed_max_s(int Npad, int n_out, int act)
+{
+    if ((act != 1 && act != 3) || (n_out != 1 && n_out != 2 && n_out != 4)
+            || (act == 3 && n_out != 2) || Npad < 16 || Npad % 16 != 0)
+        return 0;
+    const int oimg = act == 3 ? 1 : n_out;
+    const int nt = Npad / 16;
+    if (nt > 8 || nt * oimg > PSL_MAX_TILES) return 0;
+    return (PSL_LDS_CAP - psl_fixed_lds(oimg, nt, n_out)) / (4 * n_out);
+}
+
+template <int NOUT, int ACT, int NT>
+static int launch_psl_ks(
+    const uint64_t* packed, const float* diff, const float* base,
+    const float* wbg, const float* lfnull, const float* kw, const float* total,
+    const int64_t* vidx, float* phi_full, float* ey_out, int B, int S,
+    int Mpad, int M, int G, int link, hipStream_t stream)
+{
+    constexpr int OIMG = (ACT == 3) ? 1 : NOUT;
+    if constexpr (NT * OIMG > PSL_MAX_TILES) {
+        return -1;
+    } else {
+        const size_t lds = (size_t)psl_fixed_lds(OIMG, NT, NOUT)
+                           + (size_t)S * NOUT * 4;
+        if (lds > PSL_LDS_CAP) return -1;
+#define KSHAP_PSL(KSV) \
+        predict_solve_linear_packed_kernel<NOUT, ACT, NT, KSV> \
+            <<<dim3(B), dim3(256), lds, stream>>>( \
+                packed, diff, base, wbg, lfnull, kw, total, vidx, phi_full, \
+                ey_out, B, S, M, G, link)
+        switch (Mpad / 4) {
+            case 1: KSHAP_PSL(1); return 0;
+            case 2: KSHAP_PSL(2); return 0;
+            case 3: KSHAP_PSL(3); return 0;
+            default: return -1;
+        }
+#undef KSHAP_PSL
+    }
+}
+
+template <int NOUT, int ACT>
+static int launch_psl_nt(
+    const uint64_t* packed, const float* diff, const float* base,
+    const float* wbg, const float* lfnull, const float* kw, const float* total,
+    const int64_t* vidx, float* phi_full, float* ey_out, int B, int S,
+    int Mpad, int Npad, int M, int G, int link, hipStream_t stream)
+{
+#define KSHAP_PSL_NT(NTV) \
+    case NTV: \
+        return launch_psl_ks<NOUT, ACT, NTV>(packed, diff, base, wbg, lfnull, \
+            kw, total, vidx, phi_full, ey_out, B, S, Mpad, M, G, link, stream);
+    switch (Npad / 16) {
+        KSHAP_PSL_NT(1) KSHAP_PSL_NT(2) KSHAP_PSL_NT(3) KSHAP_PSL_NT(4)
+        KSHAP_PSL_NT(5) KSHAP_PSL_NT(6) KSHAP_PSL_NT(7) KSHAP_PSL_NT(8)
+    }
+#undef KSHAP_PSL_NT
+    return -1;
+}
+
+extern "C" int launch_predict_solve_linear_packed(
+    const uint64_t* packed, const float* diff, const float* base,
+    const float* wbg, const float* lfnull, const float* kw, const float* total,
+    const int64_t* vidx, float* phi_full, float* ey_out, int B, int S,
+    int Mpad, int Npad, int M, int n_out, int G, int act, int link,
+    hipStream_t stream)
+{
+    if (Mpad < 4 || Mpad > 12 || Mpad % 4 != 0 || Npad % 16 != 0 || Npad < 16
+            || Npad / 16 > 8)
+        return -1;
+    if (M < 2 || M > G || M > Mpad || (M - 1) + n_out > 16) return -1;
+    if (link != 0 && (link != 1 || lfnull == nullptr)) return -1;
+    if (S <= 0) return -1;
+    if (S > predict_solve_linear_packed_max_s(Npad, n_out, act)) return -1;
+    if (B <= 0) return 0;
+#define KSHAP_PSL_CALL(NO, ACTV) \
+    return launch_psl_nt<NO, ACTV>(packed, diff, base, wbg, lfnull, kw, total, \
+        vidx, phi_full, ey_out, B, S, Mpad, Npad, M, G, link, stream)
+    if (act == 3) {
+        if (n_out == 2) KSHAP_PSL_CALL(2, 3);
+        return -1;
+    }
+    if (act != 1) return -1;
+    switch (n_out) {
+        case 1: KSHAP_PSL_CALL(1, 1);
+        case 2: KSHAP_PSL_CALL(2, 1);
+        case 4: KSHAP_PSL_CALL(4, 1);
+        default: return -1;
+    }
+#undef KSHAP_PSL_CALL
+}
+
 
 __global__ __launch_bounds__(256)
 void varying_keys_kernel(
```

After: 6.685 million explanations/s (median of 6 runs). +2.5%, better.
